# symek/facedeform

Measured on AMD Instinct MI355X. Metric: deformed Mverts/sec at 256 ctrl pts, 1/2/4/8 MI355X vs host-CPU ref, higher is better.
Workload: dtype f32

## Files before the change

### facedeform_amd/_build.py

```python
from __future__ import annotations

import os
import shutil
import subprocess

_PKG = os.path.dirname(os.path.abspath(__file__))
_ROOT = os.path.dirname(_PKG)
CSRC = os.path.join(_PKG, "csrc")
LIB_DIR = os.path.join(_PKG, "lib")
LIB_PATH = os.path.join(LIB_DIR, "libfacedeform_hip.so")
SOURCES = ["fd_eval.hip", "fd_eval_shared.hip", "fd_build.hip", "fd_nullspace.hip", "fd_build_reg.hip", "fd_build_ml_shared.hip", "fd_build_qnn_shared.hip", "fd_capi.hip", "fd_morph.hip", "fd_capture.hip", "fd_vectors.hip", "fd_invert.hip", "fd_adjoint.hip", "fd_adjoint_points.hip", "fd_adjoint_shot.hip", "fd_adjoint_points_shot.hip", "fd_gram.hip", "fd_bake.hip", "fd_vectors_shared.hip", "fd_eval_shared64.hip", "fd_vectors_shared64.hip", "fd_eval_shared_ml.hip", "fd_vectors_shared_ml.hip", "fd_eval_shared_ml64.hip", "fd_vectors_shared_ml64.hip", "fd_sop_host.cpp"]
EXTRA_FLAGS = {"fd_eval.hip": ["-mllvm", "-amdgpu-mfma-vgpr-form"],
               "fd_eval_shared.hip": ["-fno-slp-vectorize"],
               "fd_eval_shared_ml.hip": ["-fno-slp-vectorize"],
               "fd_vectors_shared64.hip": ["-mllvm", "-disable-machine-licm"],
               "fd_vectors_shared_ml64.hip": ["-mllvm", "-disable-machine-licm"],
               "fd_adjoint_shot.hip": ["-mllvm", "-disable-machine-licm"],
               "fd_adjoint_points.hip": ["-mllvm", "-disable-machine-licm"],
               "fd_adjoint_points_shot.hip": ["-mllvm", "-disable-machine-licm"]}
HEADERS = [os.path.join(CSRC, "fd_internal.h"), os.path.join(CSRC, "fd_tuning.h"), os.path.join(CSRC, "fd_pack.h"), os.path.join(CSRC, "fd_eval_common.h"), os.path.join(CSRC, "fd_transport.h"), os.path.join(CSRC, "fd_eval_point.h"), os.path.join(CSRC, "fd_shot_launch.h"), os.path.join(CSRC, "fd_vectors_shot.h"), os.path.join(CSRC, "fd_shared64.h"), os.path.join(CSRC, "fd_shared_ml64.h"), os.path.join(CSRC, "fd_shared_ml.h"), os.path.join(CSRC, "fd_shared_common.h"), os.path.join(CSRC, "fd_shared_plan.h"), os.path.join(CSRC, "fd_shared_solve.h"), os.path.join(CSRC, "fd_shot_dev.h"), os.path.join(CSRC, "fd_fit_host.h"), os.path.join(CSRC, "fd_owned.h"), os.path.join(CSRC, "fd_operator.h"), os.path.join(CSRC, "fd_adjoint_points_shot.h"), os.path.join(CSRC, "fd_bake_plan.h"), os.path.join(_ROOT, "include", "facedeform_hip.h")]


def hipcc_path() -> str:
    for cand in (os.environ.get("HIPCC"), shutil.which("hipcc"), "/opt/rocm/bin/hipcc"):
        if cand and os.path.exists(cand):
            return cand
    raise RuntimeError("hipcc not found (set HIPCC or install ROCm)")


def is_stale() -> bool:
    if not os.path.exists(LIB_PATH):
        return True
    t = os.path.getmtime(LIB_PATH)
    deps = [os.path.join(CSRC, s) for s in SOURCES] + HEADERS
    return any(os.path.getmtime(d) > t for d in deps)


def build(force: bool = False, verbose: bool = False) -> str:
    if not force and not is_stale():
        return LIB_PATH
    os.makedirs(LIB_DIR, exist_ok=True)
    obj_dir = os.path.join(_PKG, "build")
    os.makedirs(obj_dir, exist_ok=True)
    cc = hipcc_path()
    common = ["--offload-arch=gfx950", "-O3", "-std=c++17", "-fPIC", "-ffp-contract=off", "-I", os.path.join(_ROOT, "include")]
    common += os.environ.get("FD_EXTRA_HIPCC_FLAGS", "").split()
    objs = []
    procs = []
    for src in SOURCES:
        obj = os.path.join(obj_dir, os.path.splitext(src)[0] + ".o")
        objs.append(obj)
        cmd = [cc] + common + EXTRA_FLAGS.get(src, []) + ["-x", "hip", "-c", os.path.join(CSRC, src), "-o", obj]
        if verbose:
            print(" ".join(cmd))
        procs.append((src, subprocess.Popen(cmd, stdout=subprocess.PIPE, stderr=subprocess.STDOUT)))
    for src, p in procs:
        out, _ = p.communicate()
        if p.returncode != 0:
            raise RuntimeError(f"hipcc failed on {src}:\n{out.decode(errors='replace')}")
    tmp = LIB_PATH + ".tmp"
    link = [cc, "--offload-arch=gfx950", "-shared", "-fPIC", "-o", tmp] + objs
    subprocess.check_call(link)
    os.replace(tmp, LIB_PATH)
    return LIB_PATH


if __name__ == "__main__":
    print(build(force=True, verbose=True))
```

### facedeform_amd/csrc/fd_build_reg.hip

```cpp
#include <cstdio>
#include <cstdlib>

#include "fd_internal.h"
#include "fd_pack.h"

namespace fd {

namespace {

typedef double double4_t __attribute__((ext_vector_type(4)));

constexpr double kEps = 2.220446049250313e-16;
constexpr int kRegThreads = 512;
constexpr int kRegWaves = kRegThreads / 64;
constexpr int kMaxBlocks = 16;
constexpr int kWorkers = 7;
constexpr int kSlots = 20;
constexpr int kPitch = 17;
constexpr int kTileLds = 16 * kPitch;

__device__ __forceinline__ double readlane_f64(double v, int src_lane)
{
    const long long b = __double_as_longlong(v);
    const unsigned lo = (unsigned)__builtin_amdgcn_readlane((int)(b & 0xffffffffll), src_lane);
    const unsigned hi = (unsigned)__builtin_amdgcn_readlane((int)(b >> 32), src_lane);
    return __longlong_as_double((long long)(((unsigned long long)hi << 32) | lo));
}

__device__ __forceinline__ int opaque_s(int v)
{
    asm volatile("" : "+s"(v));
    return v;
}

template <int CTRL>
__device__ __forceinline__ double dpp_f64(double v)
{
    const long long b = __double_as_longlong(v);
    const unsigned lo = (unsigned)__builtin_amdgcn_update_dpp(0, (int)(b & 0xffffffffll), CTRL, 0xf, 0xf, false);
    const unsigned hi = (unsigned)__builtin_amdgcn_update_dpp(0, (int)(b >> 32), CTRL, 0xf, 0xf, false);
    return __longlong_as_double((long long)(((unsigned long long)hi << 32) | lo));
}
__device__ __forceinline__ double wave_sum(double v)
{
    const double4_t zero = {0.0, 0.0, 0.0, 0.0};
    const double4_t d = __builtin_amdgcn_mfma_f64_16x16x4f64(v, 1.0, zero, 0, 0, 0);
    const double t = (d[0] + d[1]) + (d[2] + d[3]);
    const double4_t e = __builtin_amdgcn_mfma_f64_16x16x4f64(t, 1.0, zero, 0, 0, 0);
    return e[0];
}
__device__ __forceinline__ double wave_max(double v)
{
    double o;
    o = dpp_f64<0x121>(v); v = o > v ? o : v;
    o = dpp_f64<0x122>(v); v = o > v ? o : v;
    o = dpp_f64<0x124>(v); v = o > v ? o : v;
    o = dpp_f64<0x128>(v); v = o > v ? o : v;
    const double a = readlane_f64(v, 0), b = readlane_f64(v, 16), c = readlane_f64(v, 32), d = readlane_f64(v, 48);
    const double ab = a > b ? a : b, cd = c > d ? c : d;
    return ab > cd ? ab : cd;
}

__device__ __forceinline__ void wave_lds_sync()
{
    __builtin_amdgcn_fence(__ATOMIC_RELEASE, "wavefront");
    __builtin_amdgcn_wave_barrier();
    __builtin_amdgcn_fence(__ATOMIC_ACQUIRE, "wavefront");
}

__device__ __forceinline__ double rsqrt_nr(double d)
{
    const double y0 = __builtin_amdgcn_rsq(d);
    const double t = d * y0;
    const double e = fma(-t, y0, 1.0);
    double p = fma(e, 0.375, 0.5);
    p = p * e;
    return fma(y0, p, y0);
}

__device__ __forceinline__ double log_pos(double x)
{
    double m = __builtin_amdgcn_frexp_mant(x);
    int e = __builtin_amdgcn_frexp_exp(x);
    if (m < 0.70710678118654752) { m *= 2.0; e -= 1; }
    const double num = m - 1.0, den = m + 1.0;
    double r = __builtin_amdgcn_rcp(den);
    r = fma(fma(-den, r, 1.0), r, r);
// ... 45 lines not shown
    L.cen = p; p += 3 * kRows;
    L.V = p; p += 4 * kRows;
    L.W = p; p += 4 * kRows;
    L.F = p; p += 3 * kRows;
    L.B21 = p; p += 4 * kRows;
    L.small = p; p += kSmallDoubles;
    const size_t overlay = (size_t)kMaxBlocks * kTileLds + (size_t)(kMaxBlocks + 1) * kTileLds;
    const size_t ypart = (size_t)kRegWaves * 4 * kRows;
    L.minv = p; L.P = p + (size_t)kMaxBlocks * kTileLds; L.ypart = p;
    p += overlay > ypart ? overlay : ypart;
    L.scr = p; p += (size_t)kRegWaves * 2 * kTileLds;
    L.Z = p; p += 3 * 256;
    L.Y = p; p += 3 * 256;
    L.stat = p; p += 8;
    L.D = p; p += kTileLds;
    L.tab = reinterpret_cast<int *>(p);
    L.flag = L.tab + 300;
    return L;
}

__device__ __forceinline__ double4_t factor_invert_tile(double4_t Tt, int lane, double &piv)
{
    const int c = lane & 15, g = lane >> 4;
    piv = 0.0;
    double4_t U;
#pragma unroll
    for (int i = 0; i < 4; ++i) U[i] = (g + 4 * i == c) ? 1.0 : 0.0;
#pragma unroll
    for (int b = 0; b < 4; ++b) {
        double s[4][4];
#pragma unroll
        for (int p = 0; p < 4; ++p)
#pragma unroll
            for (int q = 0; q <= p; ++q) s[p][q] = readlane_f64(Tt[b], 4 * b + q + 16 * p);
        double l[4][4], inv[4], dk[4];
#pragma unroll
        for (int k = 0; k < 4; ++k) {
            double d = s[k][k];
#pragma unroll
            for (int e = 0; e < k; ++e) d = fma(-l[k][e], l[k][e], d);
            dk[k] = d;
            inv[k] = rsqrt_nr(d);
#pragma unroll
            for (int p = k + 1; p < 4; ++p) {
                double v = s[p][k];
#pragma unroll
                for (int e = 0; e < k; ++e) v = fma(-l[p][e], l[k][e], v);
                l[p][k] = v * inv[k];
            }
        }
#pragma unroll
        for (int k = 0; k < 4; ++k) piv = c == 4 * b + k ? dk[k] : piv;
        double m[4][4];
#pragma unroll
        for (int q = 0; q < 4; ++q) {
            m[q][q] = inv[q];
#pragma unroll
            for (int p = q + 1; p < 4; ++p) {
                double v = 0.0;
#pragma unroll
                for (int e = q; e < p; ++e) v = fma(l[p][e], m[e][q], v);
                m[p][q] = -v * inv[p];
            }
        }
        double aop = 0.0;
#pragma unroll
        for (int p = 0; p < 4; ++p)
#pragma unroll
            for (int q = 0; q <= p; ++q) aop = (c == p && g == q) ? m[p][q] : aop;
        const double4_t zero = {0.0, 0.0, 0.0, 0.0};
        const double4_t rt = __builtin_amdgcn_mfma_f64_16x16x4f64(aop, Tt[b], zero, 0, 0, 0);
        const double4_t ru = __builtin_amdgcn_mfma_f64_16x16x4f64(aop, U[b], zero, 0, 0, 0);
        const double mult = c > 4 * b + 3 ? -rt[0] : 0.0;
        Tt = __builtin_amdgcn_mfma_f64_16x16x4f64(mult, rt[0], Tt, 0, 0, 0);
        U = __builtin_amdgcn_mfma_f64_16x16x4f64(mult, ru[0], U, 0, 0, 0);
        U[b] = ru[0];
        Tt[b] = rt[0];
    }
    return U;
}

constexpr int kAff = 64;
struct PackLds {
    const double *cen, *dlt, *sol, *aff;
    const float *dl_global;
    double R;
    int sing, dup;
    __device__ __forceinline__ double centre(int j, int q) const { return cen[3 * j + q]; }
    __device__ __forceinline__ bool has_delta() const { return true; }
    __device__ __forceinline__ double delta(int j, int q) const { return dlt ? dlt[3 * j + q] : (double)dl_global[3 * j + q]; }
    __device__ __forceinline__ double weight(int j, int c) const { return sol[c * 256 + j]; }
    __device__ __forceinline__ double affine(int cc, int k, int, int T) const { return k < T ? aff[3 * k + cc] : 0.0; }
    __device__ __forceinline__ double radius(int) const { return R; }
    __device__ __forceinline__ int sing_flag() const { return sing; }
    __device__ __forceinline__ int dup_flag() const { return dup; }
};

__device__ __forceinline__ double lds_where(bool cond, const double *p, int i_true)
{
    const double v = p[cond ? i_true : 0];
    return cond ? v : 0.0;
}

__device__ __forceinline__ void assemble_tile(const double *cen, int I, int J, int c, int g, int M, int kind, double lambda, double inv_r2,
                                              double (&e)[4], double &amax_w, bool &dup)
{
    const int col = 16 * J + c;
    const double cx = cen[3 * col], cy = cen[3 * col + 1], cz = cen[3 * col + 2];
    double d2[4];
#pragma unroll
    for (int i = 0; i < 4; ++i) {
        const int row = 16 * I + g + 4 * i;
        const double dx = cen[3 * row] - cx, dy = cen[3 * row + 1] - cy, dz = cen[3 * row + 2] - cz;
        d2[i] = dx * dx + dy * dy + dz * dz;
    }
    if (kind == FD_KERNEL_THIN_PLATE) {
#pragma unroll
        for (int i = 0; i < 4; ++i) {
            const bool pos = d2[i] > 0.0;
            const double lg = log_pos(pos ? d2[i] : 1.0);
            e[i] = pos ? 0.5 * d2[i] * lg : 0.0;
        }
    } else {
#pragma unroll
        for (int i = 0; i < 4; ++i) e[i] = phi_reg(kind, d2[i], inv_r2);
    }
#pragma unroll
    for (int i = 0; i < 4; ++i) {
        const int row = 16 * I + g + 4 * i;
        const bool real = row < M && col < M;
        if (row == col) e[i] += lambda;
        else if (d2[i] == 0.0 && real) dup = true;
        if (!real) e[i] = 0.0;
        const double ae = fabs(e[i]);
        amax_w = ae > amax_w ? ae : amax_w;
    }
}

__device__ __forceinline__ void reflect_wave(const RegLds &L, int M, int T, int lane)
{
    bool singular = false;
    double cn[4] = {0.0, 0.0, 0.0, 0.0};
    double v[4][4], f[4][3];
#pragma unroll
    for (int q = 0; q < 4; ++q) {
        const int i = lane + 64 * q;
        const bool in = i < M;
        const int ic = in ? i : 0;
        const double p[4] = {1.0, L.cen[3 * ic], L.cen[3 * ic + 1], L.cen[3 * ic + 2]};
#pragma unroll
        for (int t = 0; t < 4; ++t) {
            v[q][t] = (in && t < T) ? p[t] : 0.0;
            if (in) cn[t] = fma(v[q][t], v[q][t], cn[t]);
        }
#pragma unroll
        for (int e = 0; e < 3; ++e) { const double d = L.F[e * kRows + ic]; f[q][e] = in ? d : 0.0; }
    }
#pragma unroll
    for (int t = 0; t < 4; ++t) cn[t] = wave_sum(cn[t]);
#pragma unroll
    for (int k = 0; k < 4; ++k) {
        if (k >= T) break;
        const int piv = M - 1 - k;
        const int pl = __builtin_amdgcn_readfirstlane(piv & 63), pq = __builtin_amdgcn_readfirstlane(piv >> 6);
        double rowv[4], rowf[3];
#define FD_PIVOT_ROW(Q) { _Pragma("unroll") for (int t = 0; t < 4; ++t) rowv[t] = readlane_f64(v[Q][t], pl); \
                          _Pragma("unroll") for (int e = 0; e < 3; ++e) rowf[e] = readlane_f64(f[Q][e], pl); }
        if (pq == 0) FD_PIVOT_ROW(0) else if (pq == 1) FD_PIVOT_ROW(1) else if (pq == 2) FD_PIVOT_ROW(2) else FD_PIVOT_ROW(3)
#undef FD_PIVOT_ROW
        double acc[7] = {0.0, 0.0, 0.0, 0.0, 0.0, 0.0, 0.0};
        double x[4];
#pragma unroll
        for (int q = 0; q < 4; ++q) {
// ... 101 lines not shown

__device__ __forceinline__ void gram_wave(const RegLds &L, int M, int lane)
{
    double Sm[16];
#pragma unroll
    for (int q = 0; q < 16; ++q) Sm[q] = 0.0;
#pragma unroll
    for (int q = 0; q < 4; ++q) {
        const int i = lane + 64 * q;
        if (i < M) {
#pragma unroll
            for (int a = 0; a < 4; ++a)
#pragma unroll
                for (int b = 0; b < 4; ++b) Sm[4 * a + b] = fma(L.V[4 * i + a], L.W[4 * i + b], Sm[4 * a + b]);
        }
    }
#pragma unroll
    for (int q = 0; q < 16; ++q) Sm[q] = wave_sum(Sm[q]);
    double Tm[16], ST[16], Gm[16];
#pragma unroll
    for (int q = 0; q < 16; ++q) Tm[q] = L.small[kTm + q];
#pragma unroll
    for (int a = 0; a < 4; ++a)
#pragma unroll
        for (int b = 0; b < 4; ++b) {
            double v = 0.0;
#pragma unroll
            for (int cc = 0; cc < 4; ++cc) v = fma(0.5 * (Sm[4 * a + cc] + Sm[4 * cc + a]), Tm[4 * cc + b], v);
            ST[4 * a + b] = v;
        }
#pragma unroll
    for (int a = 0; a < 4; ++a)
#pragma unroll
        for (int b = 0; b < 4; ++b) {
            double v = 0.0;
#pragma unroll
            for (int cc = 0; cc < 4; ++cc) v = fma(Tm[4 * cc + a], ST[4 * cc + b], v);
            Gm[4 * a + b] = v;
        }
#pragma unroll
    for (int a = 0; a < 4; ++a)
#pragma unroll
        for (int b = a + 1; b < 4; ++b) { const double m = 0.5 * (Gm[4 * a + b] + Gm[4 * b + a]); Gm[4 * a + b] = m; Gm[4 * b + a] = m; }
    if (lane < 16) {
        double v = 0.0;
#pragma unroll
        for (int q = 0; q < 16; ++q) v = lane == q ? Gm[q] : v;
        L.small[kGm + lane] = v;
    }
}

__device__ __forceinline__ void w_row(const RegLds &L, int i)
{
    double y[4], v[4], w[4];
#pragma unroll
    for (int t = 0; t < 4; ++t) { y[t] = L.W[4 * i + t]; v[t] = L.V[4 * i + t]; }
#pragma unroll
    for (int b = 0; b < 4; ++b) {
        double z = 0.0, h = 0.0;
#pragma unroll
        for (int a = 0; a < 4; ++a) { z = fma(y[a], L.small[kTm + 4 * a + b], z); h = fma(v[a], L.small[kGm + 4 * a + b], h); }
        w[b] = fma(-0.5, h, z);
    }
#pragma unroll
    for (int t = 0; t < 4; ++t) L.W[4 * i + t] = w[t];
}

__device__ __forceinline__ int tile_owner(int I, int J)
{
    constexpr unsigned long long kOffsets = 0x8a3ad602e31bull;
    auto w0 = [](int K) { return (K + 1 + (int)((kOffsets >> (3 * K)) & 7ull)) % kWorkers; };
    if (I == J) return J == 0 ? 0 : w0(J - 1);
    const int j = I - J - 1;
    return j == 0 ? w0(J) : (w0(J) + 1 + (j - 1) % 6) % kWorkers;
}

constexpr int kFacTiles = kMaxBlocks * (kMaxBlocks + 1) / 2;
constexpr size_t kFacL = 0, kFacMinv = (size_t)kFacTiles * 256, kFacV = kFacMinv + (size_t)kMaxBlocks * kTileLds, kFacB21 = kFacV + 4 * kRows,
                 kFacSmall = kFacB21 + 4 * kRows, kFacMeta = kFacSmall + kSmallDoubles, kFacDoubles = kFacMeta + 8;

constexpr int kFront1Tiles = kWorkers;
constexpr int kFront2Tiles = kRegWaves;
constexpr size_t kFrV = 0, kFrF = 4 * kRows, kFrB21 = 7 * kRows, kFrSmall = 11 * kRows, kFrMeta = kFrSmall + kSmallDoubles,
                 kFrTile = kFrMeta + 8, kFrY = kFrTile + 2 * (size_t)(kMaxBlocks * (kMaxBlocks + 1) / 2);
__host__ __device__ inline size_t reg_front_doubles(int M)
{
    const int nbk = (M + 15) / 16;
    return kFrY + (size_t)(nbk * (nbk + 1) / 2) * 128;
}
__device__ __forceinline__ int tile_number(int I, int J, int nbk) { return J * nbk - J * (J - 1) / 2 + (I - J); }

constexpr int kFrontMaxTpw = 4;
__global__ __launch_bounds__(kRegThreads) void k_reg_front1(const BatchSlot *tab, const PointSrc src, int use_src, int M, int T, int kind,
                                                             double lambda, double gauss_R, int tpw)
{
    const BatchSlot &slot = tab[blockIdx.z];
    __shared__ __attribute__((aligned(16))) double s_mem[10 * kRows + kSmallDoubles + 8 + kWorkers * kTileLds];
    RegLds L{};
    L.cen = s_mem; L.V = L.cen + 3 * kRows; L.F = L.V + 4 * kRows; L.small = L.F + 3 * kRows; L.stat = L.small + kSmallDoubles; L.scr = L.stat + 8;
    const int tid = threadIdx.x, lane = tid & 63;
    const int wave = __builtin_amdgcn_readfirstlane(tid >> 6);
    const int c = lane & 15, g = lane >> 4;
    const int nbk = (M + 15) / 16, ntiles = nbk * (nbk + 1) / 2;
    const bool first = blockIdx.x == 0;
    {
        const float *rest = use_src ? src.rest[blockIdx.z] : slot.rest;
        const float *delta = use_src ? src.delta[blockIdx.z] : slot.delta;
        for (int i = tid; i < M; i += kRegThreads) {
#pragma unroll
            for (int q = 0; q < 3; ++q) {
                const float r = rest[3 * i + q], d = delta[3 * i + q];
                L.cen[3 * i + q] = (double)r;
                L.F[q * kRows + i] = (double)d;
                if (first) {
                    slot.centres[3 * i + q] = (double)r;
                    if (use_src) { slot.rest[3 * i + q] = r; slot.delta[3 * i + q] = d; }
                }
            }
            if (first) slot.radii[i] = gauss_R;
        }
        for (int e = tid; e < 4 * kRows; e += kRegThreads) {
            if (e >= 4 * M || T == 0) L.V[e] = 0.0;
            if (e < 3 * kRows && e % kRows >= M) L.F[e] = 0.0;
            if (e < 3 * kRows && e >= 3 * M) L.cen[e] = 0.0;
        }
        if (tid < kSmallDoubles) L.small[tid] = 0.0;
        if (tid == 0) L.stat[3] = 0.0;
    }
    __syncthreads();
    gdouble *fr = as_global(slot.ns);
    double e[kFrontMaxTpw][4];
    int tI[kFrontMaxTpw], tJ[kFrontMaxTpw];
    bool have[kFrontMaxTpw];
    if (wave < kWorkers) {
        gdouble *stage = as_global(slot.A);
        const double inv_r2 = 1.0 / (gauss_R * gauss_R);
#pragma unroll
        for (int t = 0; t < kFrontMaxTpw; ++t) {
            const int q = ((int)blockIdx.x * tpw + t) * kFront1Tiles + wave;
            have[t] = t < tpw && q < ntiles;
            tI[t] = tJ[t] = 0;
#pragma unroll
            for (int i = 0; i < 4; ++i) e[t][i] = 0.0;
            if (have[t]) {
                int r = q, J = 0;
                while (r >= nbk - J) { r -= nbk - J; ++J; }
                tI[t] = J + r; tJ[t] = J;
                double amax_w = 0.0;
                bool dup = false;
                assemble_tile(L.cen, tI[t], tJ[t], c, g, M, kind, lambda, inv_r2, e[t], amax_w, dup);
#pragma unroll
                for (int i = 0; i < 4; ++i) stage[((size_t)q * 4 + i) * 64 + lane] = e[t][i];
                amax_w = wave_max(amax_w);
                const bool any_dup = __any(dup);
                if (lane == 0) { fr[kFrTile + 2 * q] = amax_w; fr[kFrTile + 2 * q + 1] = any_dup ? 1.0 : 0.0; }
            }
        }
    } else {
#pragma unroll
        for (int t = 0; t < kFrontMaxTpw; ++t) have[t] = false;
        if (T > 0) reflect_wave(L, M, T, lane);
    }
    __threadfence_block();
    __syncthreads();
    if (T > 0) {
#pragma unroll
        for (int t = 0; t < kFrontMaxTpw; ++t) {
            if (!have[t]) continue;
            const int q = ((int)blockIdx.x * tpw + t) * kFront1Tiles + wave;
            const int I = tI[t], J = tJ[t];
            gdouble *yq = fr + kFrY + (size_t)q * 128;
            double *sb = L.scr + (size_t)wave * kTileLds;
            if (I != J) {
                wave_lds_sync();
#pragma unroll
                for (int i = 0; i < 4; ++i) sb[(g + 4 * i) * kPitch + c] = e[t][i];
            }
            {
                double4_t acc = {0.0, 0.0, 0.0, 0.0};
#pragma unroll
                for (int s2 = 0; s2 < 4; ++s2) {
                    const double b = lds_where(c < 4, L.V, 4 * (16 * I + 4 * s2 + g) + c);
                    acc = __builtin_amdgcn_mfma_f64_16x16x4f64(e[t][s2], b, acc, 0, 0, 0);
                }
                if (c < 4) {
#pragma unroll
                    for (int i = 0; i < 4; ++i) yq[(g + 4 * i) * 4 + c] = acc[i];
                }
            }
            if (I != J) {
                wave_lds_sync();
                double4_t acc = {0.0, 0.0, 0.0, 0.0};
#pragma unroll
                for (int s2 = 0; s2 < 4; ++s2) {
                    const double a = sb[c * kPitch + 4 * s2 + g];
                    const double b = lds_where(c < 4, L.V, 4 * (16 * J + 4 * s2 + g) + c);
                    acc = __builtin_amdgcn_mfma_f64_16x16x4f64(a, b, acc, 0, 0, 0);
                }
                if (c < 4) {
#pragma unroll
                    for (int i = 0; i < 4; ++i) yq[64 + (g + 4 * i) * 4 + c] = acc[i];
                }
            }
        }
    }
    if (first && wave == kWorkers) {
        for (int x = lane; x < 4 * kRows; x += 64) fr[kFrV + x] = L.V[x];
        for (int x = lane; x < 3 * kRows; x += 64) fr[kFrF + x] = L.F[x];
        for (int x = lane; x < kSmallDoubles; x += 64) fr[kFrSmall + x] = L.small[x];
        if (lane == 0) fr[kFrMeta + 2] = L.stat[3];
    }
}

__global__ __launch_bounds__(kRegThreads) void k_reg_front2(const BatchSlot *tab, int M, int T, int tpw)
{
    const BatchSlot &slot = tab[blockIdx.z];
    __shared__ __attribute__((aligned(16))) double s_mem[8 * kRows + kSmallDoubles];
    RegLds L{};
    L.V = s_mem; L.W = L.V + 4 * kRows; L.small = L.W + 4 * kRows;
    const int tid = threadIdx.x, lane = tid & 63;
    const int wave = __builtin_amdgcn_readfirstlane(tid >> 6);
    const int c = lane & 15, g = lane >> 4;
    const int n1 = M - T;
    const int nbk = (M + 15) / 16, ntiles = nbk * (nbk + 1) / 2;
    gdouble *fr = as_global(slot.ns);
    for (int x = tid; x < 4 * kRows; x += kRegThreads) {
        L.V[x] = fr[kFrV + x];
        const int i = x >> 2, t = x & 3, r = i >> 4, row = i & 15;
        double y = 0.0;
        if (T > 0 && r < nbk) {
            gcdouble *yp = fr + kFrY + row * 4 + t;
            double v[kMaxBlocks];
#pragma unroll
            for (int k = 0; k < kMaxBlocks; ++k) {
                const int kk = k < nbk ? k : nbk - 1;
                const size_t at = kk < r ? (size_t)tile_number(r, kk, nbk) * 128 + 64 : (size_t)tile_number(kk, r, nbk) * 128;
                v[k] = yp[at];
            }
#pragma unroll
            for (int k = 0; k < kMaxBlocks; ++k) y += k < nbk ? v[k] : 0.0;
        }
        L.W[x] = y;
    }
    if (tid < kSmallDoubles) L.small[tid] = fr[kFrSmall + tid];
    if (blockIdx.x == 0 && wave == 1) {
        double amax = 0.0, dup = 0.0;
        for (int q = lane; q < ntiles; q += 64) {
            const double a = fr[kFrTile + 2 * q], d = fr[kFrTile + 2 * q + 1];
            amax = a > amax ? a : amax; dup = d > dup ? d : dup;
        }
        amax = wave_max(amax); dup = wave_max(dup);
        if (lane == 0) { fr[kFrMeta + 0] = amax; fr[kFrMeta + 1] = dup; }
    }
    __syncthreads();
    if (T > 0) {
        if (wave == 0) gram_wave(L, M, lane);
        __syncthreads();
        if (tid < kRows) w_row(L, tid);
        __syncthreads();
    }
    gdouble *stage = as_global(slot.A);
    for (int t = 0; t < tpw; ++t) {
        const int q = ((int)blockIdx.x * tpw + t) * kFront2Tiles + wave;
        if (q >= ntiles) break;
        int I = 0, J = 0;
        {
            int r = q;
            while (r >= nbk - J) { r -= nbk - J; ++J; }
            I = J + r;
        }
        double4_t S;
#pragma unroll
        for (int i = 0; i < 4; ++i) S[i] = stage[((size_t)q * 4 + i) * 64 + lane];
        if (T > 0) {
            const int ri = 16 * I + c, rj = 16 * J + c;
            const double vi = L.V[4 * ri + g], wi = L.W[4 * ri + g];
            const double vj = L.V[4 * rj + g], wj = L.W[4 * rj + g];
            S = __builtin_amdgcn_mfma_f64_16x16x4f64(-vi, wj, S, 0, 0, 0);
            S = __builtin_amdgcn_mfma_f64_16x16x4f64(-wi, vj, S, 0, 0, 0);
        }
#pragma unroll
        for (int i = 0; i < 4; ++i) {
            const int row = 16 * I + g + 4 * i, col = 16 * J + c;
            if (row >= n1 && row < M && col < n1) fr[kFrB21 + 4 * col + (M - 1 - row)] = S[i];
            if (row >= n1 || col >= n1) S[i] = row == col ? 1.0 : 0.0;
            stage[((size_t)q * 4 + i) * 64 + lane] = S[i];
        }
    }
}

template <bool FRONT>
__global__ __launch_bounds__(kRegThreads) void k_build_reg(const BatchSlot *tab, const PointSrc src, int use_src, int M, int T, int npad,
                                                            int kind, int Mpad, double lambda, double gauss_R, unsigned long long *stamps,
                                                            double *fac)
{
    const BatchSlot &slot = tab[blockIdx.z];
    extern __shared__ __attribute__((aligned(16))) double dyn_lds[];
    const RegLds L = carve(dyn_lds, M);
    const int tid = threadIdx.x, lane = tid & 63;
    const int wave = __builtin_amdgcn_readfirstlane(tid >> 6);
    const bool worker = wave < kWorkers;
    const int c = lane & 15, g = lane >> 4;
    const int n1 = M - T;
    const int nbk = (M + 15) / 16;
    const int nb = (n1 + 15) / 16;
    DevModel FD_GLOBAL *model = as_global(slot.model);
    unsigned long long st_prev = stamps ? __builtin_amdgcn_s_memtime() : 0ull;
    int st_k = 0;
#define FD_RSTAMP() if (stamps && blockIdx.z == 0 && tid == 0) { const unsigned long long t_ = __builtin_amdgcn_s_memtime(); stamps[st_k] = t_ - st_prev; atomicAdd(&stamps[84 + st_k], t_ - st_prev); if (st_k == 0) atomicAdd(&stamps[83], 1ull); ++st_k; st_prev = t_; }
    __builtin_amdgcn_s_setprio(3);

    const int ntiles = nbk * (nbk + 1) / 2;
    int nmine = 0;
    if (worker) {
        if (lane < kSlots) L.tab[wave * kSlots + lane] = 0xffff;
        wave_lds_sync();
        for (int q0 = 0; q0 < ntiles; q0 += 64) {
            int q = q0 + lane, J = 0;
            const bool in = q < ntiles;
            while (in && q >= nbk - J) { q -= nbk - J; ++J; }
            const int I = J + q;
            const bool mine = in && tile_owner(I, J) == wave;
            const unsigned long long mask = __ballot(mine);
            const int rank = nmine + __popcll(mask & ((1ull << lane) - 1ull));
            if (mine) L.tab[wave * kSlots + rank] = I | (J << 8) | ((q0 + lane) << 16);
            nmine += __popcll(mask);
        }
        nmine = __builtin_amdgcn_readfirstlane(nmine);
    }
    if constexpr (!FRONT) {
        gcdouble *fr = as_global(slot.ns);
        static_assert(4 * kRows == 2 * kRegThreads, "two entries per thread");
        double lv[2], lb[2], lf[2], ls[2], lc[2], ld[2];
#pragma unroll
        for (int h = 0; h < 2; ++h) {
            const int e = tid + kRegThreads * h;
            lv[h] = fr[kFrV + e];
            lb[h] = fr[kFrB21 + e];
            lf[h] = fr[kFrF + (e < 3 * kRows ? e : 0)];
            ls[h] = fr[kFrSmall + (e < kSmallDoubles ? e : 0)];
            lc[h] = slot.centres[e < 3 * M ? e : 0];
            ld[h] = (double)slot.delta[e < 3 * M ? e : 0];
        }
#pragma unroll
        for (int h = 0; h < 2; ++h) {
            const int e = tid + kRegThreads * h;
            L.V[e] = lv[h];
            L.B21[e] = lb[h];
            if (e < 3 * kRows) L.F[e] = lf[h];
            if (e < kSmallDoubles) L.small[e] = ls[h];
            if (e < 3 * M) { L.cen[e] = lc[h]; L.scr[e] = ld[h]; }
        }
    } else {
        const float *rest = use_src ? src.rest[blockIdx.z] : slot.rest;
        const float *delta = use_src ? src.delta[blockIdx.z] : slot.delta;
        for (int i = tid; i < M; i += kRegThreads) {
#pragma unroll
            for (int q = 0; q < 3; ++q) {
                const float r = rest[3 * i + q], d = delta[3 * i + q];
                L.cen[3 * i + q] = (double)r;
                L.F[q * kRows + i] = (double)d;
                slot.centres[3 * i + q] = (double)r;
                if (use_src) { slot.rest[3 * i + q] = r; slot.delta[3 * i + q] = d; }
            }
            slot.radii[i] = gauss_R;
        }
        for (int e = tid; e < 4 * kRows; e += kRegThreads) {
            if (e >= 4 * M) { L.V[e] = 0.0; L.W[e] = 0.0; L.B21[e] = 0.0; }
            if (e < 3 * kRows && e % kRows >= M) L.F[e] = 0.0;
            if (e < 3 * kRows && e >= 3 * M) L.cen[e] = 0.0;
        }
    }
    if (tid == 0) { L.stat[0] = INFINITY; L.stat[1] = 0.0; L.stat[2] = 0.0; L.stat[3] = FRONT ? 0.0 : as_global(slot.ns)[kFrMeta + 2]; L.flag[0] = 0; L.flag[1] = 0; L.flag[2] = 0; L.flag[3] = 0; }
    __syncthreads();
    int ijv = 0xffff;
    if (worker && lane < kSlots) ijv = L.tab[wave * kSlots + lane];
    const int ivI = ijv & 0xff, ivJ = (ijv >> 8) & 0xff;
    auto slots_where = [&](bool cond) -> unsigned { return (unsigned)__builtin_amdgcn_readfirstlane((int)(unsigned)__ballot(cond && lane < kSlots)); };
    const unsigned m_matrix = slots_where(ivI < kMaxBlocks);
#define tI(t) (opaque_s(__builtin_amdgcn_readlane(ijv, t)) & 0xff)
#define tJ(t) ((opaque_s(__builtin_amdgcn_readlane(ijv, t)) >> 8) & 0xff)
#define FD_SLOT(m, t) (((m) >> (t)) & 1u)
    FD_RSTAMP()

    if constexpr (FRONT) {
    if (worker) {
        gdouble *stage = as_global(slot.A);
        const double inv_r2 = 1.0 / (gauss_R * gauss_R);
        double amax_w = 0.0;
        bool dup = false;
#pragma nounroll
        for (int t = 0; t < nmine; ++t) {
            const int ij = __builtin_amdgcn_readfirstlane(L.tab[wave * kSlots + t]);
            const int I = ij & 0xff, J = (ij >> 8) & 0xff, q = ij >> 16;
            double e[4];
            assemble_tile(L.cen, I, J, c, g, M, kind, lambda, inv_r2, e, amax_w, dup);
#pragma unroll
            for (int i = 0; i < 4; ++i) {
                stage[((size_t)q * 4 + i) * 64 + lane] = e[i];
            }
        }
        amax_w = wave_max(amax_w);
        const bool any_dup = __any(dup);
        if (lane == 0) { L.ypart[wave] = amax_w; L.ypart[kRegWaves + wave] = any_dup ? 1.0 : 0.0; }
    } else if (T > 0) {
        reflect_wave(L, M, T, lane);
    }
    __threadfence_block();
    __syncthreads();
    }
    FD_RSTAMP()
    double amax = 0.0;
    bool dup_any = false;
    if constexpr (FRONT) {
#pragma unroll
        for (int w = 0; w < kWorkers; ++w) { amax = L.ypart[w] > amax ? L.ypart[w] : amax; dup_any = dup_any || L.ypart[kRegWaves + w] != 0.0; }
    } else {
        amax = as_global(slot.ns)[kFrMeta + 0];
        dup_any = as_global(slot.ns)[kFrMeta + 1] != 0.0;
    }
    double4_t S[kSlots];
    {
        gcdouble *stage = as_global(slot.A);
#pragma unroll
        for (int t = 0; t < kSlots; ++t) {
            const int q = __builtin_amdgcn_readlane(ijv, t) >> 16;
            S[t] = (double4_t){0.0, 0.0, 0.0, 0.0};
            if (FD_SLOT(m_matrix, t)) {
#pragma unroll
                for (int i = 0; i < 4; ++i) S[t][i] = stage[((size_t)q * 4 + i) * 64 + lane];
            }
        }
    }
    if constexpr (FRONT) {
// ... 308 lines not shown
    }
    for (int I = nb - 1; I >= 1; --I) {
        const unsigned m_row = slots_where(ivI == I && ivJ < I);
        const bool next_mine = slots_where(ivI == I && ivJ == I - 1) != 0u;
#pragma unroll
        for (int t = 0; t < kSlots; ++t) {
            if (FD_SLOT(m_row, t)) {
                double4_t acc = {0.0, 0.0, 0.0, 0.0};
                double ya[4];
#pragma unroll
                for (int s = 0; s < 4; ++s) ya[s] = lds_where(c < 3, L.Y, c * 256 + 16 * I + 4 * s + g);
                __builtin_amdgcn_sched_group_barrier(0x100, 4, 0);
                __builtin_amdgcn_sched_group_barrier(0x002, 8, 0);
                __builtin_amdgcn_sched_group_barrier(0x008, 4, 0);
#pragma unroll
                for (int s = 0; s < 4; ++s) acc = __builtin_amdgcn_mfma_f64_16x16x4f64(ya[s], S[t][s], acc, 0, 0, 0);
                if (g < 3) L.Z[g * 256 + 16 * tJ(t) + c] -= acc[0];
            }
        }
        if (next_mine) { wave_lds_sync(); solve_block(I - 1); }
        __syncthreads();
    }
    FD_RSTAMP()

    if (!worker) {
        double q12[12];
#pragma unroll
        for (int e = 0; e < 12; ++e) q12[e] = 0.0;
        double xr[4][3];
#pragma unroll
        for (int q = 0; q < 4; ++q) {
            const int i = lane + 64 * q;
            const bool in = i < n1;
            xr[q][0] = in ? L.Y[i] : 0.0; xr[q][1] = in ? L.Y[256 + i] : 0.0; xr[q][2] = in ? L.Y[512 + i] : 0.0;
            if (in && T > 0) {
#pragma unroll
                for (int k = 0; k < 4; ++k) {
                    const double b = k < T ? L.B21[4 * i + k] : 0.0;
                    q12[3 * k] = fma(b, xr[q][0], q12[3 * k]); q12[3 * k + 1] = fma(b, xr[q][1], q12[3 * k + 1]); q12[3 * k + 2] = fma(b, xr[q][2], q12[3 * k + 2]);
                }
            }
        }
        if (T > 0) {
#pragma unroll
            for (int e = 0; e < 12; ++e) q12[e] = wave_sum(q12[e]);
        }
        double a[4][3] = {};
#pragma unroll
        for (int k = 3; k >= 0; --k) {
            if (k >= T) continue;
#pragma unroll
            for (int e = 0; e < 3; ++e) {
                double v = L.small[kG + 3 * k + e] - q12[3 * k + e];
#pragma unroll
                for (int c2 = k + 1; c2 < 4; ++c2) if (c2 < T) v = fma(-L.small[kR + 4 * k + c2], a[c2][e], v);
                a[k][e] = v / L.small[kR + 4 * k + k];
            }
        }
#pragma unroll
        for (int k = 3; k >= 0; --k) {
            if (k >= T) continue;
            const int piv = M - 1 - k;
            const double tau = L.small[kTau + k];
            double d[3] = {0.0, 0.0, 0.0}, v[4];
#pragma unroll
            for (int q = 0; q < 4; ++q) {
                const int i = lane + 64 * q;
                v[q] = i <= piv ? L.V[4 * i + k] : 0.0;
#pragma unroll
                for (int e = 0; e < 3; ++e) d[e] = fma(v[q], xr[q][e], d[e]);
            }
#pragma unroll
            for (int e = 0; e < 3; ++e) d[e] = wave_sum(d[e]);
#pragma unroll
            for (int q = 0; q < 4; ++q)
#pragma unroll
                for (int e = 0; e < 3; ++e) xr[q][e] = fma(-tau * d[e], v[q], xr[q][e]);
        }
        gdouble *X = as_global(slot.X);
#pragma unroll
        for (int q = 0; q < 4; ++q) {
            const int i = lane + 64 * q;
            if (i < M) { X[i] = xr[q][0]; X[(size_t)npad + i] = xr[q][1]; X[2 * (size_t)npad + i] = xr[q][2]; }
            if (i < M) { L.Y[i] = xr[q][0]; L.Y[256 + i] = xr[q][1]; L.Y[512 + i] = xr[q][2]; }
        }
        if (lane < 12) {
            double v = 0.0;
#pragma unroll
            for (int k = 0; k < 4; ++k)
#pragma unroll
                for (int e = 0; e < 3; ++e) v = lane == 3 * k + e ? a[k][e] : v;
            L.small[kAff + lane] = v;
        }
        for (int r = M + lane; r < npad; r += 64) {
#pragma unroll
            for (int e = 0; e < 3; ++e) {
                double v = 0.0;
#pragma unroll
                for (int k = 0; k < 4; ++k) v = (r - M == k && k < T) ? a[k][e] : v;
                X[(size_t)e * npad + r] = v;
            }
        }
        if (lane == 0) {
            model->terminationtype = 0;
            model->dup_flag = dup_any ? 1 : 0;
            model->sing_flag = (L.stat[2] != 0.0 || L.stat[3] != 0.0) ? 1 : 0;
            L.stat[4] = (L.stat[2] != 0.0 || L.stat[3] != 0.0) ? 1.0 : 0.0;
            L.stat[5] = dup_any ? 1.0 : 0.0;
            model->iterations = M + T;
            model->amax_bits = (unsigned long long)__double_as_longlong(amax);
            model->pivmin_bits = (unsigned long long)__double_as_longlong(L.stat[0]);
            model->pivmax_bits = (unsigned long long)__double_as_longlong(L.stat[1]);
        }
    }
    __threadfence_block();
    __syncthreads();
    FD_RSTAMP()
    if (tid >= 256) return;
    {
        const PackLds in{L.cen, FRONT ? nullptr : L.scr, L.Y, L.small + kAff, slot.delta, gauss_R, L.stat[4] != 0.0 ? 1 : 0, L.stat[5] != 0.0 ? 1 : 0};
        packing::pack_body_from(in, slot, npad, M, Mpad, T, kind, 0, 0);
    }
    FD_RSTAMP()
    if (kind == FD_KERNEL_THIN_PLATE) {
        __syncthreads();
        for (int tile = tid >> 6; tile < Mpad / 16; tile += 4) packing::pack_tiles_body(slot, Mpad, tile, lane);
    }
    FD_RSTAMP()
#undef FD_RSTAMP
#undef tI
#undef tJ
#undef FD_SLOT
}

__global__ __launch_bounds__(256) void k_resolve_reg(const BatchSlot *tab, const PointSrc src, int use_src, int M, int T, int npad, int kind,
                                                      int Mpad, double gauss_R, const double *fac)
{
    const int fi = 1 + (int)blockIdx.z;
    const BatchSlot &slot = tab[fi];
    __shared__ double s_minv[kMaxBlocks * kTileLds];
    __shared__ double s_V[4 * kRows], s_B21[4 * kRows], s_small[kSmallDoubles];
    __shared__ double s_f[3 * kRows];
    __shared__ double s_blk[3 * 16];
    __shared__ double s_red[4 * 12];
    __shared__ double s_g[12], s_a[12];
    const int tid = threadIdx.x, lane = tid & 63;
    const int n1 = M - T, nb = (n1 + 15) / 16, nbk = (M + 15) / 16;
    gcdouble *fg = as_global(fac);
    DevModel FD_GLOBAL *model = as_global(slot.model);
    auto tile_q = [&](int I, int J) { return J * nbk - J * (J - 1) / 2 + (I - J); };
    for (int e = tid; e < kMaxBlocks * kTileLds; e += 256) s_minv[e] = fg[kFacMinv + e];
    for (int e = tid; e < 4 * kRows; e += 256) { s_V[e] = fg[kFacV + e]; s_B21[e] = fg[kFacB21 + e]; }
    if (tid < kSmallDoubles) s_small[tid] = fg[kFacSmall + tid];
    {
        const float *rest = use_src ? src.rest[fi] : slot.rest;
        const float *delta = use_src ? src.delta[fi] : slot.delta;
        for (int i = tid; i < kRows; i += 256) {
#pragma unroll
            for (int q = 0; q < 3; ++q) {
                double d = 0.0;
                if (i < M) {
                    const float r = rest[3 * i + q], dl = delta[3 * i + q];
                    d = (double)dl;
                    slot.centres[3 * i + q] = (double)r;
                    if (use_src) { slot.rest[3 * i + q] = r; slot.delta[3 * i + q] = dl; }
                }
                s_f[q * kRows + i] = d;
            }
            if (i < M) slot.radii[i] = gauss_R;
        }
    }
    __syncthreads();
    const int i0 = tid;
    for (int k = 0; k < T; ++k) {
        const int piv = M - 1 - k;
        const double v = s_V[4 * i0 + k];
        double d[3] = {v * s_f[i0], v * s_f[kRows + i0], v * s_f[2 * kRows + i0]};
        packing::block_reduce_many<3, false>(d, s_red, tid);
        const double tau = s_small[kTau + k];
#pragma unroll
        for (int e = 0; e < 3; ++e) {
            const double fv = fma(-tau * d[e], v, s_f[e * kRows + i0]);
            if (i0 == piv) { s_g[3 * k + e] = fv; s_f[e * kRows + i0] = 0.0; }
            else if (i0 < piv) s_f[e * kRows + i0] = fv;
        }
        __syncthreads();
    }
    {
        const int r = tid, I = r >> 4, rr = r & 15;
        double cur[16], nxt[16];
        auto fetch = [&](int K, double (&dst)[16]) {
            if (I > K && I < nb) {
                gcdouble *p = fg + kFacL + ((size_t)tile_q(I, K) * 4 + (rr >> 2)) * 64 + 16 * (rr & 3);
#pragma unroll
                for (int k = 0; k < 16; ++k) dst[k] = p[k];
            } else {
#pragma unroll
                for (int k = 0; k < 16; ++k) dst[k] = 0.0;
            }
        };
        fetch(0, cur);
        for (int K = 0; K < nb; ++K) {
            if (K + 1 < nb) fetch(K + 1, nxt);
            if (tid < 48) {
                const int e = tid >> 4, n = tid & 15;
                const double *mk = s_minv + (size_t)K * kTileLds;
                double z = 0.0;
#pragma unroll
                for (int k = 0; k < 16; ++k) z = fma(s_f[e * kRows + 16 * K + k], mk[n * kPitch + k], z);
                s_blk[e * 16 + n] = z;
            }
            __syncthreads();
            if (tid < 48) s_f[(tid >> 4) * kRows + 16 * K + (tid & 15)] = s_blk[tid];
            if (I > K && I < nb) {
#pragma unroll
// ... 73 lines not shown
#pragma unroll
                    for (int c2 = k + 1; c2 < 4; ++c2) if (c2 < T) v = fma(-s_small[kR + 4 * k + c2], a[c2][e], v);
                    a[k][e] = v / s_small[kR + 4 * k + k];
                }
            }
#pragma unroll
            for (int k = 0; k < 4; ++k)
#pragma unroll
                for (int e = 0; e < 3; ++e) s_a[3 * k + e] = a[k][e];
        }
        for (int k = T - 1; k >= 0; --k) {
            const int piv = M - 1 - k;
            const double v = i0 <= piv ? s_V[4 * i0 + k] : 0.0;
            double d[3] = {v * xr[0], v * xr[1], v * xr[2]};
            packing::block_reduce_many<3, false>(d, s_red, tid);
            const double tau = s_small[kTau + k];
#pragma unroll
            for (int e = 0; e < 3; ++e) xr[e] = fma(-tau * d[e], v, xr[e]);
        }
        __syncthreads();
        gdouble *X = as_global(slot.X);
        if (i0 < M) { X[i0] = xr[0]; X[(size_t)npad + i0] = xr[1]; X[2 * (size_t)npad + i0] = xr[2]; }
        for (int rrow = M + tid; rrow < npad; rrow += 256) {
#pragma unroll
            for (int e = 0; e < 3; ++e) X[(size_t)e * npad + rrow] = (rrow - M < T) ? s_a[3 * (rrow - M) + e] : 0.0;
        }
        if (tid == 0) {
            model->terminationtype = 0;
            model->dup_flag = fg[kFacMeta + 1] != 0.0 ? 1 : 0;
            model->sing_flag = fg[kFacMeta + 2] != 0.0 ? 1 : 0;
            model->iterations = M + T;
            model->amax_bits = (unsigned long long)__double_as_longlong(fg[kFacMeta + 0]);
            model->pivmin_bits = (unsigned long long)__double_as_longlong(fg[kFacMeta + 3]);
            model->pivmax_bits = (unsigned long long)__double_as_longlong(fg[kFacMeta + 4]);
        }
    }
    __threadfence_block();
    __syncthreads();
    packing::pack_body(slot, npad, M, Mpad, T, kind, 0, 0);
    if (kind == FD_KERNEL_THIN_PLATE) {
        __syncthreads();
        for (int tile = tid >> 6; tile < Mpad / 16; tile += 4) packing::pack_tiles_body(slot, Mpad, tile, lane);
    }
}

}

size_t reg_factor_doubles() { return kFacDoubles; }

bool reg_applicable(int kind, int term, double lambda, int M)
{
    return M <= 16 * kMaxBlocks && spd_applicable(kind, term, lambda, M);
}

hipError_t reg_build_init()
{
    static bool done[64] = {};
    int dev = 0;
    hipError_t e = hipGetDevice(&dev);
    if (e != hipSuccess) return e;
    if (dev >= 0 && dev < 64 && done[dev]) return hipSuccess;
    e = hipFuncSetAttribute((const void *)k_build_reg<true>, hipFuncAttributeMaxDynamicSharedMemorySize,
                            (int)(sizeof(double) * reg_lds_doubles(16 * kMaxBlocks)));
    if (e == hipSuccess)
        e = hipFuncSetAttribute((const void *)k_build_reg<false>, hipFuncAttributeMaxDynamicSharedMemorySize,
                                (int)(sizeof(double) * reg_lds_doubles(16 * kMaxBlocks)));
    if (e == hipSuccess && dev >= 0 && dev < 64) done[dev] = true;
    return e;
}

hipError_t launch_build_reg_shared(const BuildBuffers &b, hipStream_t stream, const PointSrc *src, hipEvent_t ev_mid, double *fac)
{
    static const PointSrc none{};
    if (ev_mid) (void)hipEventRecord(ev_mid, stream);
    const size_t lds = sizeof(double) * reg_lds_doubles(b.M);
    hipLaunchKernelGGL(k_build_reg<true>, dim3(1, 1, 1), dim3(kRegThreads), lds, stream, b.d_slots, src ? *src : none, src ? 1 : 0, b.M, b.T,
                       b.npad, b.kind, b.Mpad, b.lambda, b.gauss_R, (unsigned long long *)nullptr, fac);
    if (b.nbatch > 1)
        hipLaunchKernelGGL(k_resolve_reg, dim3(1, 1, (unsigned)b.nbatch - 1), dim3(256), 0, stream, b.d_slots, src ? *src : none, src ? 1 : 0,
                           b.M, b.T, b.npad, b.kind, b.Mpad, b.gauss_R, (const double *)fac);
    return hipGetLastError();
}

hipError_t launch_build_reg(const BuildBuffers &b, hipStream_t stream, const PointSrc *src, hipEvent_t ev_mid)
{
    static const PointSrc none{};
    const unsigned nbatch = (unsigned)b.nbatch;
    if (ev_mid) (void)hipEventRecord(ev_mid, stream);
    const size_t lds = sizeof(double) * reg_lds_doubles(b.M);
    static unsigned long long *d_stamps = nullptr;
    hipStreamCaptureStatus cs = hipStreamCaptureStatusNone;
    static const bool stamps_env = tuning_env("FD_REG_STAMPS") != nullptr;
    static const bool stamps_late = stamps_env && atoi(tuning_env("FD_REG_STAMPS")) == 2;
    const bool want_stamps = stamps_env && hipStreamIsCapturing(stream, &cs) == hipSuccess && cs == hipStreamCaptureStatusNone;
    if (want_stamps && !d_stamps) { (void)hipMalloc((void **)&d_stamps, 96 * sizeof(unsigned long long)); (void)hipMemset(d_stamps, 0, 96 * sizeof(unsigned long long)); }
    const bool split = b.reg_front != 0 && reg_front_doubles(b.M) <= ns_doubles(b.M);
    if (split) {
        const int nbk = (b.M + 15) / 16, ntiles = nbk * (nbk + 1) / 2;
        const int cus = (int)device_cus();
        auto tiles_per_wave = [&](int per_wg) {
            int tpw = 1;
            while (tpw < kFrontMaxTpw && ((ntiles + per_wg * tpw - 1) / (per_wg * tpw)) * (int)nbatch > cus) ++tpw;
            return tpw;
        };
        const int tpw1 = tiles_per_wave(kFront1Tiles), tpw2 = tiles_per_wave(kFront2Tiles);
        hipLaunchKernelGGL(k_reg_front1, dim3((unsigned)((ntiles + kFront1Tiles * tpw1 - 1) / (kFront1Tiles * tpw1)), 1, nbatch), dim3(kRegThreads), 0, stream,
                           b.d_slots, src ? *src : none, src ? 1 : 0, b.M, b.T, b.kind, b.lambda, b.gauss_R, tpw1);
        hipLaunchKernelGGL(k_reg_front2, dim3((unsigned)((ntiles + kFront2Tiles * tpw2 - 1) / (kFront2Tiles * tpw2)), 1, nbatch), dim3(kRegThreads), 0, stream,
                           b.d_slots, b.M, b.T, tpw2);
        hipLaunchKernelGGL(k_build_reg<false>, dim3(1, 1, nbatch), dim3(kRegThreads), lds, stream, b.d_slots, none, 0, b.M, b.T,
                           b.npad, b.kind, b.Mpad, b.lambda, b.gauss_R, want_stamps ? d_stamps : nullptr, (double *)nullptr);
    } else
    hipLaunchKernelGGL(k_build_reg<true>, dim3(1, 1, nbatch), dim3(kRegThreads), lds, stream, b.d_slots, src ? *src : none, src ? 1 : 0, b.M, b.T,
                       b.npad, b.kind, b.Mpad, b.lambda, b.gauss_R, want_stamps ? d_stamps : nullptr, (double *)nullptr);
    if (want_stamps && d_stamps && stamps_late) {
        static bool registered = false;
        static unsigned long long *d_keep = nullptr;
        d_keep = d_stamps;
        if (!registered) {
            registered = true;
            atexit([] {
                unsigned long long h[96];
                if (d_keep && hipDeviceSynchronize() == hipSuccess && hipMemcpy(h, d_keep, sizeof(h), hipMemcpyDeviceToHost) == hipSuccess && h[83]) {
                    fprintf(stderr, "[k_build_reg stamps, MEAN over %llu launches (no read-back per launch): table | assembly | tile loads | reflectors | KV | W + rotation | Cholesky | back substitution | recovery | pack]\n  ", h[83]);
                    for (int q = 0; q < 10; ++q) fprintf(stderr, " %llu", h[84 + q] / h[83]);
                    fprintf(stderr, "\n");
                }
            });
        }
    } else if (want_stamps && d_stamps) {
        unsigned long long h[80];
        (void)hipStreamSynchronize(stream);
        if (hipMemcpy(h, d_stamps, sizeof(h), hipMemcpyDeviceToHost) == hipSuccess) {
            fprintf(stderr, "[k_build_reg stamps, shader cycles: table | assembly | tile loads | reflectors + Q^T f | Y = K V | W + rotation + B21 | Cholesky | back substitution | recovery | pack]\n  ");
            for (int q = 0; q < 10; ++q) fprintf(stderr, " %llu", h[q]);
            fprintf(stderr, "\n   Cholesky steps (cycles since its start: inverse K in LDS | panel K in LDS, as wave 0 sees them):");
            for (int q = 16; q < 48; ++q) fprintf(stderr, "%s%llu", (q - 16) % 2 ? " " : "\n     ", h[q]);
            fprintf(stderr, "\n");
        }
    }
    return hipGetLastError();
}

}
```

### facedeform_amd/csrc/fd_capi.hip

```cpp
#include <algorithm>
#include <atomic>
#include <chrono>
#include <cmath>
#include <cstdarg>
#include <cstdio>
#include <cstdlib>
#include <cstring>
#include <initializer_list>
#include <new>
#include <vector>

#include "fd_fit_host.h"
#include "fd_internal.h"
#include "fd_owned.h"
#include "fd_shared_plan.h"

using namespace fd;
using namespace fd_fit;

struct GraphKey {
    int M, kind, term, nparams;
    double params[4];
    const void *A, *rest, *rec32;
};
// ... 58 lines not shown
    bool status_inflight = false;
    int sticky_rc = FD_OK;

    int64_t cap_N = 0;
    DevBuf<float> d_P, d_dist2, d_fall;
    DevBuf<float> d_tu, d_tv, d_nrm;
    DevBuf<float> d_vec, d_vecP;
    DevBuf<int> d_iters;
    DevBuf<double> d_adj;
    DevBuf<double> d_adjp;
    DevBuf<double> d_gram;
    DevBuf<double> d_bake, d_bakeout;
    DevBuf<double> d_adjs;
    DevBuf<float> d_gshot;
    size_t cap_hgshot = 0;
    float *h_gshot = nullptr;
    int64_t mesh_N = 0, mesh_cap = 0;
    bool mesh_has_dist2 = false, mesh_has_frames = false;
    DevBuf<float> m_P, m_dist2, m_tu, m_tv, m_nrm;
    DevBuf<float> m_out, m_fall;

    Event ev0, ev_mid, ev1;

    GraphExec build_exec;
    bool use_graph = true;
    GraphKey graph_key{}, resolve_key{};
    char err[512] = {0};
};

struct ShotScratch {
    DevBuf<void> d;
    Event consumed_ev;
    bool consumed = false;
    Event eval_ev;
    bool eval_pending = false;
};

struct fd_batch {
    int n = 0;
    int device = 0;
    fd_ctx *ctxs[kMaxBatch] = {};
    uint64_t gens[kMaxBatch] = {};
    DevBuf<BatchSlot> d_slots;
    PointSrc src{};
    bool have_src = false;
    Event ev0, ev_mid, ev1;
    GraphExec exec;
    bool use_graph = true;
    GraphKey key{};
    hipStream_t waited_stream = nullptr;
    Event status_ev;
    struct SharedSet {
        DevBuf<void> d_wtiles, d_frames;
        Event packed_ev;
        Event eval_ev;
        hipEvent_t eval_done = nullptr;
        bool eval_pending = false;
    } sets[2];
    Pinned<int> h_mismatch;
    int eval_cus = 0;
    int shared_factor = 0;
    DevBuf<double> d_fac;
    int last_shared_factor = 0;
    DevBuf<void> d_mlfac;
    int shared_lu = 0;
    DevBuf<void> d_qnnfac;
    bool qnn_slot_ready = false;
    int qnn_slot_M = 0, qnn_slot_npad = 0;
    int cur_set = 0;
    bool packed_valid = false;
    bool prepared = false;
    unsigned long long prep_gen[kMaxBatch] = {0};
    float *prep_P_out[kMaxBatch] = {nullptr};
    float *prep_fall[kMaxBatch] = {nullptr};
    bool prep_has_fall = false;
    Event fallback_ev;
    ShotScratch s64;
    ShotScratch sml;
    ShotScratch sml64;
    ShotScratch sadjp;
    Event group_ev;
    bool lean = false;
    hipEvent_t consumed_override = nullptr;
    char err[512] = {0};
};


static thread_local char g_err[512] = {0};

static void set_err(fd_ctx *ctx, const char *fmt, ...)
{
    char *dst = ctx ? ctx->err : g_err;
    va_list ap;
    va_start(ap, fmt);
    vsnprintf(dst, 512, fmt, ap);
    va_end(ap);
}

static hipStream_t cur_stream(fd_ctx *ctx)
{
    if (ctx->stream_) return ctx->stream_;
    if (!ctx->own_stream && ctx->own_stream.create() != hipSuccess) (void)hipGetLastError();
    return ctx->own_stream;
}

#define FD_HIP(ctx, call)                                                               \
    do {                                                                                \
        hipError_t e_ = (call);                                                         \
        if (e_ != hipSuccess) {                                                         \
            set_err(ctx, "%s failed: %s (%s:%d)", #call, hipGetErrorString(e_), __FILE__, __LINE__); \
            return FD_E_DEVICE;                                                         \
        }                                                                               \
    } while (0)

static int use_device(fd_ctx *ctx)
{
    int cur = -1;
    FD_HIP(ctx, hipGetDevice(&cur));
    if (cur != ctx->device) FD_HIP(ctx, hipSetDevice(ctx->device));
    return FD_OK;
}

constexpr bool kGrow = true;
template <typename T>
static int dev_alloc(fd_ctx *ctx, DevBuf<T> &b, size_t count, bool grow = false)
{
    const hipError_t e = grow ? b.grow(count) : b.alloc(count);
    if (e == hipSuccess) return FD_OK;
    set_err(ctx, "hipMalloc(%zu bytes) failed: %s", (count ? count : 1) * sizeof(T), hipGetErrorString(e));
    return FD_E_NOMEM;
}

static int order_of(const fd_ctx *ctx) { return ctx->M + term_cols(ctx->term); }
static int ml_layers(const fd_ctx *ctx) { return ctx->kind == FD_KERNEL_GAUSSIAN_ML ? (int)ctx->params[1] : 0; }
static int model_centres(const fd_ctx *ctx) { return ctx->kind == FD_KERNEL_GAUSSIAN_ML ? ctx->M * ml_layers(ctx) : ctx->M; }
static int eval_kind(const fd_ctx *ctx) { return ctx->kind == FD_KERNEL_GAUSSIAN_ML ? FD_KERNEL_GAUSSIAN_QNN : ctx->kind; }
static int record_layers(const fd_ctx *ctx) { return ctx->kind == FD_KERNEL_GAUSSIAN_ML ? ml_layers(ctx) : ctx->imported_layers; }

static int ensure_records_capacity(fd_ctx *ctx, int n)
{
    int rc;
    if (n > ctx->cap_records) {
        const int npad = round_up(n, kRecPad);
        if ((rc = dev_alloc(ctx, ctx->d_centres, (size_t)n * 3))) return rc;
        if ((rc = dev_alloc(ctx, ctx->d_radii, (size_t)n))) return rc;
        if ((rc = dev_alloc(ctx, ctx->d_W, (size_t)(n + 4) * 3))) return rc;
        if ((rc = dev_alloc(ctx, ctx->d_rec32, (size_t)npad))) return rc;
        if ((rc = dev_alloc(ctx, ctx->d_rec64, (size_t)npad))) return rc;
        if ((rc = dev_alloc(ctx, ctx->d_tiles, (size_t)npad / 16))) return rc;
        if ((rc = dev_alloc(ctx, ctx->d_tiles16, (size_t)npad / 16))) return rc;
        ctx->cap_records = n;
    }
    return FD_OK;
}

static int ensure_model_capacity(fd_ctx *ctx, int M)
{
    int rc;
    if (M > ctx->cap_M) {
        if ((rc = dev_alloc(ctx, ctx->d_rest, (size_t)M * 3))) return rc;
        if ((rc = dev_alloc(ctx, ctx->d_delta, (size_t)M * 3))) return rc;
        if ((rc = dev_alloc(ctx, ctx->d_ns, ns_doubles(M)))) return rc;
        ctx->cap_M = M;
    }
    return ensure_records_capacity(ctx, M);
}
// ... 1614 lines not shown
    va_end(ap);
}

fd_batch *fd_batch_create(fd_ctx *const *ctxs, int n)
{
    if (!ctxs || n <= 0 || n > kMaxBatch) { set_err(nullptr, "fd_batch_create: need 1..%d contexts", kMaxBatch); return nullptr; }
    for (int i = 0; i < n; ++i) {
        if (!ctxs[i] || ctxs[i]->device != ctxs[0]->device) { set_err(nullptr, "fd_batch_create: contexts must exist and share one device"); return nullptr; }
        for (int j = 0; j < i; ++j)
            if (ctxs[j] == ctxs[i]) { set_err(nullptr, "fd_batch_create: context listed twice"); return nullptr; }
    }
    fd_batch *b = new (std::nothrow) fd_batch();
    if (!b) { set_err(nullptr, "fd_batch_create: out of host memory"); return nullptr; }
    b->n = n;
    b->device = ctxs[0]->device;
    for (int i = 0; i < n; ++i) b->ctxs[i] = ctxs[i];
    bool ok = hipSetDevice(b->device) == hipSuccess;
    ok = ok && b->d_slots.alloc((size_t)n) == hipSuccess;
    ok = ok && b->ev0.create(hipEventDefault) == hipSuccess && b->ev_mid.create(hipEventDefault) == hipSuccess &&
         b->ev1.create(hipEventDefault) == hipSuccess;
    ok = ok && b->status_ev.create(hipEventDisableTiming) == hipSuccess;
    ok = ok && b->h_mismatch.alloc(1, hipHostMallocMapped) == hipSuccess;
    if (ok) *b->h_mismatch = 0;
    if (!ok) {
        set_err(nullptr, "fd_batch_create: device resource allocation failed: %s", hipGetErrorString(hipGetLastError()));
        fd_batch_destroy(b);
        return nullptr;
    }
    return b;
}

void fd_batch_destroy(fd_batch *b)
{
    if (!b) return;
    (void)hipSetDevice(b->device);
    for (int i = 0; i < b->n; ++i) {
        fd_ctx *c = b->ctxs[i];
        if (c && c->wait_event == b->ev1) {
            if (c->wait_stream) (void)hipStreamSynchronize(c->wait_stream);
            c->wait_event = nullptr; c->wait_stream = nullptr; c->wait_batch = nullptr;
        }
        if (c && c->tev0 == b->ev0) { c->tev0 = c->ev0; c->tev_mid = c->ev_mid; c->tev1 = c->ev1; }
        if (c && (c->status_poll == b->status_ev || c->status_poll == b->ev1)) { c->status_poll = c->status_ev; c->status_inflight = false; }
    }
    delete b;
}

const char *fd_batch_last_error(const fd_batch *b) { return b ? b->err : g_err; }

int fd_batch_set_points_dev(fd_batch *b, const float *const *d_rest_xyz, const float *const *d_delta_xyz, int M)
{
    if (!b || !d_rest_xyz || !d_delta_xyz) return FD_E_INVALID;
    if (M <= 0 || M + 4 > kMaxOrder) { batch_err(b, "fd_batch_set_points_dev: M = %d outside 1..%d", M, kMaxOrder - 4); return FD_E_INVALID; }
    b->prepared = false;
    if (b->h_mismatch && *b->h_mismatch != 0) {
        const int who = *b->h_mismatch - 1;
        *b->h_mismatch = 0;
        batch_err(b, "shared-rig evaluation of the previous group: context %d was built on other rest points than context 0 (same "
                     "address, other contents); its frame was passed through", who);
        return FD_E_INVALID;
    }
    for (int i = 0; i < b->n; ++i)
        if (!d_rest_xyz[i] || !d_delta_xyz[i]) { batch_err(b, "fd_batch_set_points_dev: null array for context %d", i); return FD_E_INVALID; }
    for (int i = 0; i < b->n; ++i) {
        fd_ctx *c = b->ctxs[i];
        int rc = use_device(c);
        if (!rc) rc = ensure_model_capacity(c, M);
        if (rc) { batch_err(b, "context %d: %s", i, c->err); return rc; }
        c->M = M;
        c->points_set = true;
        c->built = false;
        c->build_pending = false;
        c->have_factor = false;
        c->deltas_only = false;
        c->rest_src = d_rest_xyz[i];
        c->rig_build_id = 0;
        b->src.rest[i] = d_rest_xyz[i];
        b->src.delta[i] = d_delta_xyz[i];
    }
    b->have_src = true;
    return FD_OK;
}

int fd_batch_build_async(fd_batch *b, void *hip_stream)
{
    if (!b) return FD_E_INVALID;
    b->prepared = false;
    fd_ctx *c0 = b->ctxs[0];
    int rc = use_device(c0);
    if (rc) { batch_err(b, "%s", c0->err); return rc; }
    hipStream_t stream = hip_stream ? (hipStream_t)hip_stream : cur_stream(c0);
    for (int i = 0; i < b->n; ++i) {
        fd_ctx *c = b->ctxs[i];
        if (!c->points_set) { batch_err(b, "fd_batch_build: context %d has no control points", i); return FD_E_INVALID; }
        c->imported_layers = 0;
        if (!same_model(c, c0)) {
            batch_err(b, "fd_batch_build: context %d differs from context 0 in M, kernel, parameters or term", i);
            return FD_E_INVALID;
        }
    }
    const int npad = round_up(order_of(c0), 32);
    bool table_stale = false;
    for (int i = 0; i < b->n; ++i) {
        fd_ctx *c = b->ctxs[i];
        const bool grew = npad > c->cap_npad;
        if ((rc = ensure_solver_capacity(c, npad)) || (rc = ensure_records_capacity(c, model_centres(c))) || (rc = sync_slot(c))) {
            batch_err(b, "context %d: %s", i, c->err);
            return rc;
        }
        if (grew) {
            const size_t cols = (size_t)c->cap_npad + kRhsCols + 16;
            hipError_t e = hipMemsetAsync(c->d_A, 0, sizeof(double) * (size_t)c->cap_npad * cols, stream);
            if (e != hipSuccess) { batch_err(b, "hipMemsetAsync failed: %s", hipGetErrorString(e)); return FD_E_DEVICE; }
        }
        if (b->gens[i] != c->alloc_gen) table_stale = true;
    }
    if (table_stale) {
        b->qnn_slot_ready = false;
        BatchSlot tab[kMaxBatch];
        for (int i = 0; i < b->n; ++i) { tab[i] = b->ctxs[i]->h_slot; b->gens[i] = b->ctxs[i]->alloc_gen; }
        hipError_t e = hipMemcpy(b->d_slots, tab, sizeof(BatchSlot) * (size_t)b->n, hipMemcpyHostToDevice);
        if (e != hipSuccess) { batch_err(b, "slot table upload failed: %s", hipGetErrorString(e)); return FD_E_DEVICE; }
    }
    BuildBuffers bb;
    choose_build(b->ctxs, b->n, bb);
    bb.d_slots = b->d_slots;
    bb.nbatch = b->n;
    if (bb.reg && reg_build_init() != hipSuccess) { (void)hipGetLastError(); bb.reg = 0; }
    bb.reg_front = (b->eval_cus <= 0 || b->eval_cus >= (int)device_cus()) ? 1 : 0;
    bb.group_panels = b->n >= 4 ? 1 : 0;

    bool same_rest_launch = b->have_src;
    for (int i = 1; i < b->n && same_rest_launch; ++i) same_rest_launch = b->src.rest[i] == b->src.rest[0];
    bool shared_ml = b->shared_factor != 0 && bb.ml_layers > 0 && same_rest_launch && ml_shared_applies(bb.M, bb.ml_layers, b->n);
    if (shared_ml && ml_shared_init() != hipSuccess) { (void)hipGetLastError(); shared_ml = false; }
    if (shared_ml && b->d_mlfac.grow(ml_shared_scratch_bytes(bb)) != hipSuccess) { (void)hipGetLastError(); shared_ml = false; }
    bool shared_qnn = b->shared_lu != 0 && c0->kind == FD_KERNEL_GAUSSIAN_QNN && bb.ml_layers == 0 && bb.nopivot && !bb.spd &&
                      bb.npad <= 1024 && bb.M >= bb.T && same_rest_launch && qnn_shared_applies(bb.M, b->n);
    for (int i = 0; i < b->n && shared_qnn; ++i) shared_qnn = b->ctxs[i]->solver == FD_SOLVER_AUTO;
    if (shared_qnn && qnn_shared_init() != hipSuccess) { (void)hipGetLastError(); shared_qnn = false; }
    if (shared_qnn && qnn_shared_scratch_bytes(bb) > b->d_qnnfac.cap) {
        b->qnn_slot_ready = false;
        if (b->d_qnnfac.grow(qnn_shared_scratch_bytes(bb)) != hipSuccess) { (void)hipGetLastError(); shared_qnn = false; }
    }

    const GraphKey key = graph_key(c0, (bb.spd << 9) | (bb.small << 10) | (bb.reg << 11) | (bb.nopivot << 12), false);
    if (!bb.reg && !shared_ml && !shared_qnn && b->use_graph &&
        ensure_graph(stream, &b->exec, &b->key, key, [&] { return launch_build(bb, stream, nullptr); }) != hipSuccess)
        b->use_graph = false;
#define FD_BHIP(call)                                                                         \
    do {                                                                                      \
        hipError_t e_ = (call);                                                               \
        if (e_ != hipSuccess) { batch_err(b, "%s failed: %s", #call, hipGetErrorString(e_)); return FD_E_DEVICE; } \
    } while (0)
    const bool shared_fac_ok = same_rest_launch;
    bool shared_fac = b->shared_factor != 0 && bb.reg && shared_fac_ok && b->n > 1;
    if (shared_fac && !b->d_fac && b->d_fac.alloc(reg_factor_doubles()) != hipSuccess) {
        (void)hipGetLastError(); shared_fac = false;
    }
    b->last_shared_factor = (shared_fac || shared_ml || shared_qnn) ? 1 : 0;
    if (!b->lean) FD_BHIP(hipEventRecord(b->ev0, stream));
    if (shared_fac) {
        FD_BHIP(launch_build_reg_shared(bb, stream, &b->src, nullptr, b->d_fac));
        b->have_src = false;
    } else if (bb.reg) {
        FD_BHIP(launch_build_reg(bb, stream, b->have_src ? &b->src : nullptr, nullptr));
        b->have_src = false;
    } else {
    FD_BHIP(launch_prepare(bb, stream, b->have_src ? &b->src : nullptr));
    b->have_src = false;
    if (shared_ml) {
        FD_BHIP(hipEventRecord(b->ev_mid, stream));
        FD_BHIP(launch_build_ml_shared(bb, stream, b->d_mlfac));
    } else if (shared_qnn) {
        FD_BHIP(hipEventRecord(b->ev_mid, stream));
        const bool fill = !(b->qnn_slot_ready && b->qnn_slot_M == bb.M && b->qnn_slot_npad == bb.npad);
        b->qnn_slot_ready = false;
        FD_BHIP(launch_build_qnn_shared(bb, stream, b->d_qnnfac, fill));
        b->qnn_slot_ready = true; b->qnn_slot_M = bb.M; b->qnn_slot_npad = bb.npad;
    } else if (b->use_graph && b->exec) {
        FD_BHIP(hipEventRecord(b->ev_mid, stream));
        FD_BHIP(hipGraphLaunch(b->exec, stream));
    } else {
        FD_BHIP(launch_build(bb, stream, b->ev_mid));
    }
    }
    if (!b->lean) FD_BHIP(hipEventRecord(b->ev1, stream));
    b->waited_stream = nullptr;
#undef FD_BHIP
    static std::atomic<uint64_t> build_ids{0};
    const uint64_t this_build = same_rest_launch ? ++build_ids : 0;
    hipEvent_t t0 = b->lean ? nullptr : b->ev0, t_mid = b->lean ? nullptr : (bb.reg ? b->ev0 : b->ev_mid), t1 = b->lean ? nullptr : b->ev1;
    for (int i = 0; i < b->n; ++i) note_build_enqueued(b->ctxs[i], b->ev1, stream, b, t0, t_mid, t1, &bb, this_build);
    if (shared_qnn)
        for (int i = 0; i < b->n; ++i) b->ctxs[i]->have_factor = false;
    arm_status(b->ctxs, b->n, stream, bb.reg != 0, b->ev1, b->status_ev);
    return FD_OK;
}

static int batch_poll(fd_batch *b)
{
    if (b->h_mismatch && *b->h_mismatch != 0) {
        batch_err(b, "shared-rig evaluation: context %d was built on other rest points than context 0 (same address, other "
                     "contents); its frame was passed through", *b->h_mismatch - 1);
        return FD_E_INVALID;
    }
    bool any = false;
    for (int i = 0; i < b->n; ++i) any = any || b->ctxs[i]->status_inflight || b->ctxs[i]->sticky_rc != FD_OK;
    if (!any) return FD_OK;
    bool shared_pending = false;
    hipEvent_t shared_ev = nullptr;
    for (int i = 0; i < b->n; ++i)
        if (b->ctxs[i]->status_inflight && (b->ctxs[i]->status_poll == b->status_ev || b->ctxs[i]->status_poll == b->ev1)) {
            shared_pending = true; shared_ev = b->ctxs[i]->status_poll;
        }
    if (shared_pending) {
        const hipError_t q = hipEventQuery(shared_ev);
        if (q == hipErrorNotReady) { (void)hipGetLastError(); return FD_OK; }
    }
    for (int i = 0; i < b->n; ++i) {
        const bool lu_before = b->ctxs[i]->prefer_lu;
        const int rc = poll_status(b->ctxs[i]);
        if (b->ctxs[i]->prefer_lu != lu_before) b->prepared = false;
        if (rc) { batch_err(b, "context %d: %s", i, b->ctxs[i]->err); return rc; }
    }
    return FD_OK;
}

int fd_batch_build_result(fd_batch *b, fd_report *reports)
{
    if (!b) return FD_E_INVALID;
    int first = FD_OK;
    for (int i = 0; i < b->n; ++i) {
        const int rc = fd_build_result(b->ctxs[i], reports ? &reports[i] : nullptr);
        if (rc && !first) { first = rc; batch_err(b, "context %d: %s", i, b->ctxs[i]->err); }
    }
    return first;
}

int fd_solve_operator(fd_ctx *ctx, double *S)
{
    if (!ctx || !S) return FD_E_INVALID;
    if (!ctx->points_set) { set_err(ctx, "fd_solve_operator: no control points (call fd_set_points first)"); return FD_E_NOT_BUILT; }
    int rc = use_device(ctx);
    if (rc) return rc;
    FD_HIP(ctx, hipStreamSynchronize(cur_stream(ctx)));
    const int M = ctx->M, rows = model_centres(ctx) + 4;
    const int builds = (M + 2) / 3;
    const int nh = builds < kMaxBatch ? builds : kMaxBatch;
    fd_ctx *helpers[kMaxBatch] = {};
    DevBuf<float> d_unit;
    fd_batch *batch = nullptr;
    auto done = [&](int code) {
        if (batch) fd_batch_destroy(batch);
        for (fd_ctx *h : helpers) if (h) fd_destroy(h);
        d_unit.reset();
        return code;
    };
    fd_config cfg{};
    cfg.struct_size = (int)sizeof(cfg);
    cfg.device = ctx->device; cfg.eval_precision = ctx->eval_precision; cfg.solver = ctx->solver;
    for (int i = 0; i < nh; ++i) {
        fd_ctx *h = helpers[i] = fd_create(&cfg);
        if (!h) { set_err(ctx, "fd_solve_operator: %s", g_err); return done(FD_E_NOMEM); }
        if ((rc = fd_set_kernel(h, ctx->kind, ctx->params, ctx->nparams)) || (rc = fd_set_term(h, ctx->term))) {
            set_err(ctx, "fd_solve_operator: %s", h->err);
            return done(rc);
        }
        h->prefer_lu = ctx->prefer_lu;
        h->stream_ = cur_stream(ctx);
    }
    const size_t per = (size_t)M * 3;
    if (d_unit.alloc(per * (size_t)nh) != hipSuccess) {
        (void)hipGetLastError();
        set_err(ctx, "fd_solve_operator: hipMalloc(%zu bytes) failed", sizeof(float) * per * (size_t)nh);
        return done(FD_E_NOMEM);
    }
    std::vector<float> unit(per * (size_t)nh);
    std::vector<double> W((size_t)rows * 3);
// ... 316 lines not shown
    sc.consumed = true;
    sc.eval_pending = record_eval(sc.eval_ev, stream);
}

static void shot_vectors_evaluated(ShotScratch &sc, hipStream_t stream)
{
    if (sc.eval_pending && hipEventRecord(sc.eval_ev, stream) == hipSuccess) return;
    (void)hipGetLastError();
    (void)hipStreamSynchronize(stream);
}

static bool one_build(const fd_batch *b)
{
    const uint64_t id = b->ctxs[0]->rig_build_id;
    if (id == 0) return false;
    for (int i = 1; i < b->n; ++i)
        if (b->ctxs[i]->rig_build_id != id) return false;
    return true;
}

static int vectors_per_context(fd_batch *b, hipStream_t stream, int precision, hipEvent_t consumed_ev, int64_t N, const float *d_P_in,
                               float *const *d_P_out, const float *d_dist2, float *const *d_falloff_out, const float *d_tu,
                               const float *d_tv, const float *d_nrm, float radius2, float falloffrate, const fd_batch_vectors *vec)
{
    for (int i = 0; i < b->n; ++i) {
        DeformArgs a = deform_args(b->ctxs[i], Mesh{N, d_P_in, d_dist2, d_tu, d_tv, d_nrm, radius2, falloffrate}, d_P_out[i],
                                   d_falloff_out ? d_falloff_out[i] : nullptr);
        a.precision = precision;
        const VectorArgs v{vec->N, vec->tu, vec->tv, vec->N ? vec->N_out[i] : nullptr, vec->tu ? vec->tu_out[i] : nullptr,
                           vec->tv ? vec->tv_out[i] : nullptr, vec->jacobian ? vec->jacobian[i] : nullptr};
        hipError_t e = launch_vectors(a, v, stream);
        if (e != hipSuccess) { batch_err(b, "launch_vectors failed: %s", hipGetErrorString(e)); return FD_E_DEVICE; }
    }
    if (hipEventRecord(consumed_ev, stream) != hipSuccess) { (void)hipGetLastError(); return FD_E_DEVICE; }
    return FD_OK;
}

static int shared_pack(fd_batch *b, hipStream_t stream, int ek, float *const *d_P_out, float *const *d_falloff_out)
{
    fd_ctx *c0 = b->ctxs[0];
    const int si = b->packed_valid ? (b->cur_set ^ 1) : 0;
    fd_batch::SharedSet &st = b->sets[si];
    SharedDeformArgs a{};
    a.N = 1; a.Mpad = round_up(c0->M, kRecPad); a.nF = b->n; a.kind = ek; a.ctiles = c0->d_tiles16;
    a.falloff_out = d_falloff_out;
    int rc;
    if (!b->lean && (rc = batch_poll(b))) return rc;
    for (int i = 0; i < b->n; ++i) {
        fd_ctx *c = b->ctxs[i];
        a.rec32[i] = c->d_rec32; a.model[i] = c->d_model; a.P_out[i] = d_P_out[i]; a.centres[i] = c->d_centres;
        if ((rc = order_after_batch(c, stream))) { batch_err(b, "context %d: %s", i, c->err); return rc; }
    }
    if (one_build(b)) for (int i = 1; i < b->n; ++i) a.centres[i] = a.centres[0];
    const SharedPlan pl = shared_plan(a.Mpad, a.nF, a.kind);
    const size_t wb = pl.wtile_bytes, fb = pl.frame_bytes;
    if (wb > st.d_wtiles.cap || fb > st.d_frames.cap) {
        st.d_wtiles.reset(); st.d_frames.reset(); st.eval_pending = false;
        if (st.d_wtiles.grow(wb) != hipSuccess || st.d_frames.grow(fb) != hipSuccess) {
            (void)hipGetLastError();
            batch_err(b, "shared-rig evaluation: scratch allocation (%zu bytes) failed", wb + fb);
            return FD_E_NOMEM;
        }
    }
    if ((rc = wait_last_eval(b, "shared-rig evaluation", stream, &st.eval_pending, st.eval_done))) return rc;
    a.wtiles = st.d_wtiles; a.frames = st.d_frames;
    a.packed_ev = b->lean ? nullptr : (st.packed_ev.make() ? st.packed_ev : nullptr);
    b->consumed_override = nullptr;
    a.mode = 1;
    a.M = c0->M;
    if (b->h_mismatch && hipHostGetDevicePointer((void **)&a.mismatch, b->h_mismatch, 0) != hipSuccess) { (void)hipGetLastError(); a.mismatch = nullptr; }
    hipError_t e = launch_deform_shared(a, stream);
    if (e != hipSuccess) { batch_err(b, "launch_deform_shared (pack) failed: %s", hipGetErrorString(e)); return FD_E_DEVICE; }
    b->cur_set = si;
    b->packed_valid = b->lean || st.packed_ev != nullptr;
    b->prepared = true;
    for (int i = 0; i < b->n; ++i) {
        b->prep_P_out[i] = d_P_out[i]; b->prep_fall[i] = d_falloff_out ? d_falloff_out[i] : nullptr;
        b->prep_gen[i] = b->ctxs[i]->model_gen;
    }
    b->prep_has_fall = d_falloff_out != nullptr;
    return FD_OK;
}

int fd_batch_prepare_shared(fd_batch *b, void *hip_stream, float *const *d_P_out, float *const *d_falloff_out)
{
    if (!b || !d_P_out) return FD_E_INVALID;
    fd_ctx *c0 = b->ctxs[0];
    int rc = use_device(c0);
    if (rc) { batch_err(b, "%s", c0->err); return rc; }
    hipStream_t stream = hip_stream ? (hipStream_t)hip_stream : cur_stream(c0);
    int ek = 0;
    const int applies = shared_applies(b, "fd_batch_prepare_shared", d_P_out, &ek);
    if (applies < 0) return applies;
    if (applies == 0) return FD_OK;
    return shared_pack(b, stream, ek, d_P_out, d_falloff_out);
}

int fd_batch_deform_shared_dev(fd_batch *b, void *hip_stream, int64_t N, const float *d_P_in, float *const *d_P_out,
                               const float *d_dist2, float *const *d_falloff_out, const float *d_tu,
                               const float *d_tv, const float *d_nrm, float radius2, float falloffrate)
{
    if (!b || !d_P_out) return FD_E_INVALID;
    int rc = shot_check_mesh(b, "fd_batch_deform_shared_dev", N, d_P_in, d_tu, d_tv, d_nrm);
    if (rc) return rc;
    if (N == 0) return FD_OK;
    fd_ctx *c0 = b->ctxs[0];
    rc = use_device(c0);
    if (rc) { batch_err(b, "%s", c0->err); return rc; }
    hipStream_t stream = hip_stream ? (hipStream_t)hip_stream : cur_stream(c0);
    int ek = 0;
    const int applies = shared_applies(b, "fd_batch_deform_shared_dev", d_P_out, &ek);
    if (applies < 0) return applies;
    if (applies == 0) {
        const float *pin[kMaxBatch], *pd2[kMaxBatch], *ptu[kMaxBatch], *ptv[kMaxBatch], *pnr[kMaxBatch];
        for (int i = 0; i < b->n; ++i) { pin[i] = d_P_in; pd2[i] = d_dist2; ptu[i] = d_tu; ptv[i] = d_tv; pnr[i] = d_nrm; }
        rc = fd_batch_deform_dev(b, hip_stream, N, pin, d_P_out, d_dist2 ? pd2 : nullptr, d_falloff_out, d_tu ? ptu : nullptr,
                                 d_tu ? ptv : nullptr, d_tu ? pnr : nullptr, radius2, falloffrate);
        if (rc == FD_OK && b->fallback_ev.make()) {
            if (hipEventRecord(b->fallback_ev, stream) != hipSuccess) { (void)hipGetLastError(); rc = FD_E_DEVICE; }
            b->packed_valid = false;
            b->consumed_override = nullptr;
        }
        return rc;
    }
    bool reuse = b->prepared && b->prep_has_fall == (d_falloff_out != nullptr);
    for (int i = 0; reuse && i < b->n; ++i)
        reuse = b->prep_P_out[i] == d_P_out[i] && (!d_falloff_out || b->prep_fall[i] == d_falloff_out[i]) &&
                b->prep_gen[i] == b->ctxs[i]->model_gen;
    if (reuse) {
        if (!b->lean && (rc = batch_poll(b))) return rc;
        if (!b->prepared) reuse = false;
        for (int i = 0; reuse && i < b->n; ++i)
            if ((rc = order_after_batch(b->ctxs[i], stream))) { batch_err(b, "context %d: %s", i, b->ctxs[i]->err); return rc; }
    }
    if (reuse) {
        fd_batch::SharedSet &ps = b->sets[b->cur_set];
        if (!b->lean && ps.packed_ev && hipStreamWaitEvent(stream, ps.packed_ev, 0) != hipSuccess) {
            batch_err(b, "fd_batch_deform_shared_dev: hipStreamWaitEvent failed: %s", hipGetErrorString(hipGetLastError()));
            return FD_E_DEVICE;
        }
    } else if ((rc = shared_pack(b, stream, ek, d_P_out, d_falloff_out))) {
        return rc;
    }
    fd_batch::SharedSet &st = b->sets[b->cur_set];
    SharedDeformArgs a{};
    a.N = N; a.P_in = d_P_in; a.dist2 = d_dist2; a.tu = d_tu; a.tv = d_tv; a.nrm = d_nrm;
    a.radius2 = radius2; a.falloffrate = falloffrate;
    a.Mpad = round_up(c0->M, kRecPad); a.nF = b->n;
    a.ctiles = c0->d_tiles16;
    a.kind = ek;
    a.falloff_out = d_falloff_out;
    for (int i = 0; i < b->n; ++i) { a.rec32[i] = b->ctxs[i]->d_rec32; a.model[i] = b->ctxs[i]->d_model; a.P_out[i] = d_P_out[i]; }
    a.wtiles = st.d_wtiles; a.frames = st.d_frames;
    a.packed_ev = nullptr;
    a.mode = 2;
    a.delta_out = c0->output == FD_OUTPUT_DISPLACEMENT;
    a.max_wgs = b->eval_cus;
    hipError_t e = launch_deform_shared(a, stream);
    if (e != hipSuccess) { batch_err(b, "launch_deform_shared failed: %s", hipGetErrorString(e)); return FD_E_DEVICE; }
    if (b->lean) {
        st.eval_done = b->ev1;
        st.eval_pending = true;
    } else {
        st.eval_pending = record_eval(st.eval_ev, stream);
        st.eval_done = st.eval_ev;
    }
// ... 397 lines not shown
    if (b->n < shared_vectors_ml64_min_frames(ml_layers(c0))) {
        return vectors_per_context(b, stream, FD_EVAL_FP64, b->sml64.consumed_ev, N, d_P_in, d_P_out, d_dist2, d_falloff_out, d_tu, d_tv, d_nrm,
                                   radius2, falloffrate, vec);
    }
    SharedVectorMl64Args a{};
    fill_mesh(a, N, d_P_in, d_dist2, d_tu, d_tv, d_nrm, radius2, falloffrate);
    a.M = c0->M; a.layers = ml_layers(c0); a.nF = b->n;
    fill_vector_tables(a, b->n, vec);
    a.scratch = b->sml64.d;
    a.max_wgs = b->eval_cus;
    hipError_t e = launch_vectors_shared_ml64(a, stream);
    if (e != hipSuccess) { batch_err(b, "launch_vectors_shared_ml64 failed: %s", hipGetErrorString(e)); return FD_E_DEVICE; }
    shot_vectors_evaluated(b->sml64, stream);
    return FD_OK;
}

const char *fd_shared_vectors_ml_fp64_kernel_name(int M, int layers, int frames)
{
    return shared_vectors_ml64_kernel_name(M, layers, frames);
}

int fd_batch_wait_consumed(fd_batch *b, void *hip_stream)
{
    if (!b) return FD_E_INVALID;
    hipEvent_t ev = b->consumed_override ? b->consumed_override : (b->packed_valid ? b->sets[b->cur_set].packed_ev : b->fallback_ev);
    hipEvent_t evs[5] = {ev, nullptr, nullptr, nullptr, nullptr};
    int n_ev = ev ? 1 : 0;
    for (const ShotScratch *sc : {&b->s64, &b->sml, &b->sml64, &b->sadjp})
        if (sc->consumed) evs[n_ev++] = sc->consumed_ev;
    if (n_ev == 0) return FD_OK;
    fd_ctx *c0 = b->ctxs[0];
    int rc = use_device(c0);
    if (rc) { batch_err(b, "%s", c0->err); return rc; }
    hipStream_t stream = hip_stream ? (hipStream_t)hip_stream : cur_stream(c0);
    for (int i = 0; i < n_ev; ++i)
        if (hipStreamWaitEvent(stream, evs[i], 0) != hipSuccess) {
            batch_err(b, "fd_batch_wait_consumed: hipStreamWaitEvent failed: %s", hipGetErrorString(hipGetLastError()));
            return FD_E_DEVICE;
        }
    return FD_OK;
}

int fd_batch_cook_group(fd_batch *b, void *build_stream, void *eval_stream, const float *d_rest_xyz,
                        const float *const *d_delta_xyz, int M, int64_t N, const float *d_P_in, float *const *d_P_out,
                        float *const *d_falloff_out, const fd_group_events *events)
{
    if (!b || !d_rest_xyz || !d_delta_xyz || !d_P_out) return FD_E_INVALID;
    fd_ctx *c0 = b->ctxs[0];
    hipStream_t bs = build_stream ? (hipStream_t)build_stream : cur_stream(c0);
    hipStream_t es = eval_stream ? (hipStream_t)eval_stream : bs;
    auto mark = [&](void *ev, hipStream_t st) { if (ev && hipEventRecord((hipEvent_t)ev, st) != hipSuccess) (void)hipGetLastError(); };
#ifdef FD_TUNING
    static const bool cook_timing = tuning_env("FD_COOK_TIMING") != nullptr;
    struct CookClock {
        bool on; double t[6]; int n = 0;
        static double now() { timespec ts; clock_gettime(CLOCK_MONOTONIC, &ts); return ts.tv_sec * 1e6 + ts.tv_nsec * 1e-3; }
        void tick() { if (on && n < 6) t[n++] = now(); }
        ~CookClock() { if (on && n == 6) fprintf(stderr, "[cook_group host us] wait_consumed %.1f | set_points %.1f | build %.1f | packing %.1f | evaluation %.1f\n", t[1] - t[0], t[2] - t[1], t[3] - t[2], t[4] - t[3], t[5] - t[4]); }
    } clk{cook_timing};
#define FD_COOK_TICK() clk.tick()
#else
#define FD_COOK_TICK()
#endif
    FD_COOK_TICK();
    int rc = fd_batch_wait_consumed(b, build_stream);
    if (rc) return rc;
    FD_COOK_TICK();
    const float *rest[kMaxBatch];
    for (int i = 0; i < b->n; ++i) rest[i] = d_rest_xyz;
    if ((rc = fd_batch_set_points_dev(b, rest, d_delta_xyz, M))) return rc;
    const bool lean = es == bs;
    struct LeanScope {
        fd_batch *b; hipStream_t s; bool on, built = false;
        ~LeanScope() {
            if (!on) return;
            if (built && hipEventRecord(b->ev1, s) != hipSuccess) (void)hipGetLastError();
            b->prepared = false;
            b->lean = false;
        }
    } scope{b, bs, lean};
    b->lean = lean;
    FD_COOK_TICK();
    if (events) mark(events->before_build, bs);
    if ((rc = fd_batch_build_async(b, build_stream))) return rc;
    scope.built = true;
    if (events) mark(events->after_build, bs);
    FD_COOK_TICK();
    if ((rc = fd_batch_prepare_shared(b, build_stream, d_P_out, d_falloff_out))) return rc;
    FD_COOK_TICK();
    if (es != bs) {
        if (!b->group_ev.make() || hipEventRecord(b->group_ev, bs) != hipSuccess || hipStreamWaitEvent(es, b->group_ev, 0) != hipSuccess) {
            batch_err(b, "fd_batch_cook_group: ordering the evaluation stream failed: %s", hipGetErrorString(hipGetLastError()));
            return FD_E_DEVICE;
        }
    }
    if (events) mark(events->before_eval, es);
    rc = fd_batch_deform_shared_dev(b, es, N, d_P_in, d_P_out, nullptr, d_falloff_out, nullptr, nullptr, nullptr, 1.0f, 1.0f);
    if (events) mark(events->after_eval, es);
    FD_COOK_TICK();
    if (lean && rc == FD_OK && b->packed_valid && b->sets[b->cur_set].eval_pending) b->consumed_override = b->ev1;
    return rc;
}

int fd_batch_set_eval_cus(fd_batch *b, int n_cus)
{
    if (!b) return FD_E_INVALID;
    b->eval_cus = n_cus > 0 ? n_cus : 0;
    return FD_OK;
}

int fd_batch_set_shared_factor(fd_batch *b, int on)
{
    if (!b) return FD_E_INVALID;
    b->shared_factor = on ? 1 : 0;
    return FD_OK;
}

int fd_batch_last_build_shared_factor(const fd_batch *b) { return b ? b->last_shared_factor : 0; }

const char *fd_shared_ml_build_kernel_name(int M, int layers, int frames) { return ml_shared_kernel_name(M, layers, frames); }

int fd_batch_set_shared_lu(fd_batch *b, int on)
{
    if (!b) return FD_E_INVALID;
    b->shared_lu = on ? 1 : 0;
    return FD_OK;
}

const char *fd_shared_qnn_build_kernel_name(int M, int frames) { return qnn_shared_kernel_name(M, frames); }

int fd_batch_size(const fd_batch *b) { return b ? b->n : 0; }

const char *fd_shared_kernel_name(int M, int frames, int kind)
{
    const bool takes = (kind == FD_KERNEL_THIN_PLATE || kind == FD_KERNEL_GAUSSIAN || kind == FD_KERNEL_GAUSSIAN_QNN) && M > 0 && round_up(M, kRecPad) >= 32 &&
                       frames >= 1 && frames <= kMaxBatch;
    return takes ? shared_plan(round_up(M, kRecPad), frames, kind).kernel : "";
}

}

#include "fd_shot_dev.h"

struct fd_shot_dev {
    fd_ctx *engine = nullptr;
    Stream work, copy;
    DevBuf<float> d_rig;
    int M = 0, F = 0;
    DevBuf<float> d_vecs;
    const float *v_in[3] = {nullptr, nullptr, nullptr};
    struct Set {
        DevBuf<float> d;
        Event eval_ev, delivered_ev;
        bool delivering = false;
    } sets[2];
    int set_frames = 0;
    int64_t set_Np = 0;
    bool set_fall = false;
    int set_nvec = 0;
    char err[512] = {0};
};

static void shot_err(fd_shot_dev *sd, const char *fmt, ...)
{
    va_list ap;
    va_start(ap, fmt);
    vsnprintf(sd->err, sizeof(sd->err), fmt, ap);
    va_end(ap);
}

static int shot_failed(fd_shot_dev *sd, const char *call, hipError_t e)
// ... 272 lines not shown
```

### facedeform_amd/csrc/fd_eval_shared.hip

```cpp
#include <cstdio>
#include <cstdlib>

#include <type_traits>

#include "fd_eval_common.h"
#include "fd_shared_common.h"
#include "fd_shared_plan.h"

namespace fd {

namespace {


static_assert(sizeof(MfmaTileH) == kMfmaTileHBytes && sizeof(SharedFrame) == kSharedFrameBytes, "fd_shared_plan.h is sized by these");

struct SharedOut {
    float *P_out[kMaxBatch];
    float *falloff_out[kMaxBatch];
};

struct SharedParams {
    int64_t N;
    const float *P_in;
    const float *dist2;
    const float *tu, *tv, *nrm;
    float radius2, falloffrate;
    int ntiles;
    int nkb;
    int nF, nT;
    int kchunk;
    const MfmaTileH *ctiles;
    const float *norm;
    const uint4 *wtiles;
    const SharedFrame *frames;
    int fast;
    int delta;
    unsigned long long *stamps;
};

struct SharedSlots {
    const Rec32 *rec32[kMaxBatch];
    const DevModel *model[kMaxBatch];
    const double *centres[kMaxBatch];
    int M;
    int nreal;
    int *mismatch;
};

__device__ __forceinline__ bool rig_matches(const SharedSlots &slots, int f, int nF, int l, int per)
{
    bool same = true;
    if (f > 0 && f < nF && slots.centres[f] != slots.centres[0]) {
        const double *a = slots.centres[f], *b0 = slots.centres[0];
        const int n = 3 * slots.M;
        bool diff = false;
        int e = l;
        for (; e + 7 * per < n; e += 8 * per) {
            double va[8], vb[8];
#pragma unroll
            for (int u = 0; u < 8; ++u) { va[u] = a[e + u * per]; vb[u] = b0[e + u * per]; }
#pragma unroll
            for (int u = 0; u < 8; ++u) diff |= !(va[u] == vb[u]);
        }
        for (; e < n; e += per) diff |= !(a[e] == b0[e]);
        same = !diff;
    }
    for (int off = per / 2; off >= 1; off >>= 1) same = (__shfl_xor((int)same, off) != 0) && same;
    if (!same && l == 0 && slots.mismatch) *slots.mismatch = (f < slots.nreal ? f : slots.nreal - 1) + 1;
    return same;
}

__global__ __launch_bounds__(256) void k_pack_shared(const SharedSlots slots, const SharedOut out, int nF, int Mpad, int dense,
                                                      uint4 *wtiles, SharedFrame *frames, const MfmaTileH *ctiles, int gauss,
                                                      size_t poly_at, size_t copy_at, size_t norm_at)
{
    const int kb = blockIdx.x, T = blockIdx.y, nT = gridDim.y;
    constexpr int per = (int)(sizeof(MfmaTileH) / 16);
    uint4 *copy = wtiles + copy_at;
    if (T == 0 && gauss) {
        if (threadIdx.x < 32) {
            const int centre = 32 * kb + (int)threadIdx.x;
            copy[(size_t)2 * kb * per + threadIdx.x] =
                centre < Mpad ? *reinterpret_cast<const uint4 *>(&slots.rec32[0][centre]) : make_uint4(0u, 0u, 0u, 0u);
        }
    } else if (T == 0) {
        const int ntiles = Mpad / 16;
        if ((int)threadIdx.x < 2 * per) {
            const int tile = 2 * kb + (int)threadIdx.x / per;
            copy[(size_t)2 * kb * per + threadIdx.x] =
// ... 377 lines not shown
                normalize3(u[0], u[1], u[2]);
                normalize3(v[0], v[1], v[2]);
                normalize3(n[0], n[1], n[2]);
                float gm[3][3];
#pragma unroll
                for (int r = 0; r < 3; ++r)
#pragma unroll
                    for (int c = 0; c < 3; ++c) gm[r][c] = u[r] * u[c] + v[r] * v[c] + n[r] * n[c];
#pragma unroll
                for (int c = 0; c < 3; ++c) {
                    a1[c] = u[0] * gm[0][c] + u[1] * gm[1][c] + u[2] * gm[2][c];
                    a2[c] = v[0] * gm[0][c] + v[1] * gm[1][c] + v[2] * gm[2][c];
                }
                normalize3(a1[0], a1[1], a1[2]);
                normalize3(a2[0], a2[1], a2[2]);
            }
        }
#pragma unroll
        for (int fs = 0; fs < kSlots; ++fs) {
            {
                const int f = fs;
                if (f >= p.nF) continue;
                const float inv = __uint_as_float((unsigned)__builtin_amdgcn_readlane((int)tab[(8 * f) / 64], (8 * f) % 64));
                const bool built = __builtin_amdgcn_readlane((int)tab[(8 * f + 1) / 64], (8 * f + 1) % 64) != 0;
                const uint64_t pout = ((uint64_t)(unsigned)__builtin_amdgcn_readlane((int)tab[(8 * f + 5) / 64], (8 * f + 5) % 64) << 32) |
                                      (unsigned)__builtin_amdgcn_readlane((int)tab[(8 * f + 4) / 64], (8 * f + 4) % 64);
                const uint64_t fout = ((uint64_t)(unsigned)__builtin_amdgcn_readlane((int)tab[(8 * f + 7) / 64], (8 * f + 7) % 64) << 32) |
                                      (unsigned)__builtin_amdgcn_readlane((int)tab[(8 * f + 6) / 64], (8 * f + 6) % 64);
                if (!doit) continue;
                Pos3 FD_GLOBAL *dstP = (Pos3 FD_GLOBAL *)((char FD_GLOBAL *)(pout + 12ull * (uint64_t)vbase) + off12);
                if (!built) {
                    if (p.delta) store_pos3(dstP, 0.f, 0.f, 0.f);
                else if (pout != (uint64_t)p.P_in) store_pos3(dstP, pos[0], pos[1], pos[2]);
                    continue;
                }
                float disp[3];
                if constexpr (DENSE) {
                    const int B = fs / 16, k = (fs % 16) / 4, r = fs % 4;
                    disp[0] = acc[3 * B][k][r] * inv; disp[1] = acc[3 * B + 1][k][r] * inv; disp[2] = acc[3 * B + 2][k][r] * inv;
                } else {
                    const int T = fs / 4, k = fs % 4;
                    disp[0] = acc[T][k][0] * inv; disp[1] = acc[T][k][1] * inv; disp[2] = acc[T][k][2] * inv;
                }
                if (p.tu) {
                    const float da1 = disp[0] * a1[0] + disp[1] * a1[1] + disp[2] * a1[2];
                    const float da2 = disp[0] * a2[0] + disp[1] * a2[1] + disp[2] * a2[2];
#pragma unroll
                    for (int c = 0; c < 3; ++c) disp[c] = a1[c] * da1 + a2[c] * da2;
                }
                if (fout) __builtin_nontemporal_store(fall, (float FD_GLOBAL *)((char FD_GLOBAL *)(fout + 4ull * (uint64_t)vbase) + off4));
                store_pos3_nt(dstP, base[0] + disp[0] * fall, base[1] + disp[1] * fall, base[2] + disp[2] * fall);
            }
        }
        FD_SSTAMP(3)
    };
    int grp = blockIdx.x;
    bool built_here = true;
#pragma unroll
    for (int q = 0; q < kTabRegs; ++q) {
        const int idx = 64 * q + lane;
        if (idx < kSlots * 8 && (idx & 7) == 1) built_here = built_here && tab[q] != 0u;
    }
    if (p.fast && __all(built_here)) {
        const int nfull = (int)(p.N / kSharedThreads);
        for (; grp < nfull; grp += gridDim.x) do_group(grp, std::true_type{});
    }
    for (; grp < ngroups; grp += gridDim.x) do_group(grp, std::false_type{});
    if (stamp && lane == 0) {
        for (int q = 0; q < 4; ++q) p.stamps[wave * 8 + q] = st_acc[q];
    }
#undef FD_SSTAMP
}


typedef float f32x16 __attribute__((ext_vector_type(16)));

__global__ __launch_bounds__(256) void k_pack_shared_wide(const SharedSlots slots, const SharedOut out, int nF, int nslot, int Mpad,
                                                           uint4 *wtiles, SharedFrame *frames, const MfmaTileH *ctiles, int gauss, int layout,
                                                           size_t poly_at, size_t copy_at, size_t norm_at)
{
    const int kb = blockIdx.x, T = blockIdx.y, NT = gridDim.y;
    const int w16 = wide_w16(NT);
    if (T == 0) {
        uint2 *dst = reinterpret_cast<uint2 *>(wtiles + copy_at) + (size_t)kb * 128;
        if (gauss) {
            if (threadIdx.x < 32) {
                const int centre = 32 * kb + (int)threadIdx.x;
                wtiles[copy_at + (size_t)kb * 64 + threadIdx.x] =
                    centre < Mpad ? *reinterpret_cast<const uint4 *>(&slots.rec32[0][centre]) : make_uint4(0u, 0u, 0u, 0u);
            }
        } else if (layout == 1) {
            if (threadIdx.x < 64) {
                const int lane = threadIdx.x, h = lane >> 5, r = lane & 31;
                const int tile = 2 * kb + (r >> 4);
                uint4 v = make_uint4(0u, 0u, 0u, 0u);
                if (tile < Mpad / 16) {
                    const unsigned *a0 = ctiles[tile].a[16 * (2 * h) + (r & 15)], *a1 = ctiles[tile].a[16 * (2 * h + 1) + (r & 15)];
                    v = make_uint4(a0[0], a0[1], a1[0], a1[1]);
                }
                wtiles[copy_at + (size_t)kb * 64 + lane] = v;
            }
        } else if (threadIdx.x < 128) {
            const int i = threadIdx.x >> 6, lane = threadIdx.x & 63, h = lane >> 5, r = lane & 31;
            const int tile = 2 * kb + (r >> 4);
            uint2 v = make_uint2(0u, 0u);
            if (tile < Mpad / 16) { const unsigned *a = ctiles[tile].a[16 * (2 * i + h) + (r & 15)]; v = make_uint2(a[0], a[1]); }
            dst[threadIdx.x] = v;
        }
        if (kb == 0 && threadIdx.x == 255) {
            const float *nn = slots.model[0]->norm32;
            wtiles[norm_at] = make_uint4(__float_as_uint(nn[0]), __float_as_uint(nn[1]), __float_as_uint(nn[2]), __float_as_uint(nn[3]));
        }
    }
    __shared__ float s_scale[kWideSlots];
    {
        const int f = threadIdx.x >> 3, l = threadIdx.x & 7;
        float m = 0.f;
        if (f < nslot) {
            m = slots.model[f]->wmax32;
        }
        for (int off = 4; off >= 1; off >>= 1) m = fmaxf(m, __shfl_xor(m, off));
        const bool same_rig = (kb == 0 && T == 0) ? rig_matches(slots, f, nslot, l, 8) : true;
        if (l == 0) {
            int k = 0;
            if (m > 0.f && m < INFINITY) k = 13 - (__builtin_amdgcn_frexp_expf(m) - 1);
            k = k < -100 ? -100 : (k > 100 ? 100 : k);
            s_scale[f] = ldexpf(1.f, k);
            if (kb == 0 && T == 0) {
                SharedFrame fr;
                fr.inv_scale = ldexpf(1.f, -k - (gauss ? kGaussShift : 0));
                fr.built = (f < nslot && same_rig && slots.model[f]->terminationtype == 1) ? 1 : 0;
                fr.pad[0] = fr.pad[1] = 0;
                fr.P_out = f < nslot ? out.P_out[f] : nullptr;
                fr.falloff_out = f < nslot ? out.falloff_out[f] : nullptr;
                frames[f] = fr;
            }
        }
    }
    __syncthreads();
    if (threadIdx.x >= 128) return;
    const int s = threadIdx.x >> 6, lane = threadIdx.x & 63, h = lane >> 5;
    int f, c;
    if (layout == 1) {
        const int rho = lane & 31, k = 16 * T + 4 * (rho >> 3) + (rho & 3);
        f = 2 * (k / 3) + ((rho >> 2) & 1); c = k % 3;
    } else {
        const int row = 32 * T + (lane & 31);
        f = row / 3; c = row % 3;
    }
    const bool live = f < nslot;
    const float sc = live ? s_scale[f] : 0.f;
    f16x8 hi, lo;
#pragma unroll
    for (int m = 0; m < 8; ++m) {
        const int centre = 32 * kb + 8 * (2 * s + (m >> 2)) + 4 * h + (m & 3);
        float w = 0.f;
        if (live && centre < Mpad) {
            const Rec32 r = slots.rec32[f][centre];
            w = (c == 0 ? r.wx : (c == 1 ? r.wy : r.wz)) * sc;
        }
        const _Float16 hh = (_Float16)w;
        hi[m] = hh;
        lo[m] = (_Float16)(w - (float)hh);
    }
    uint4 *dst = wtiles + (size_t)kb * w16 + (size_t)((T * 2 + s) * 2) * 64;
    dst[lane] = __builtin_bit_cast(uint4, hi);
    dst[64 + lane] = __builtin_bit_cast(uint4, lo);
    if (kb == 0 && s == 0) {
        f16x8 pt;
#pragma unroll
        for (int m = 0; m < 8; ++m) {
            const int coef = h == 0 ? (m < 5 ? m : m - 4) : (m == 0 ? 4 : (m < 6 ? m - 1 : -1));
            const bool want_lo = h == 1 && m >= 1;
            float w = 0.f;
            if (live && coef >= 0) w = slots.model[f]->poly32[5 * c + coef] * sc;
            const _Float16 hh = (_Float16)w;
            pt[m] = want_lo ? (_Float16)(w - (float)hh) : hh;
        }
        wtiles[poly_at + (size_t)T * 64 + lane] = __builtin_bit_cast(uint4, pt);
    }
}

constexpr int kWideVpm = 3;
constexpr int kW1Vpm = 3;

template <bool GAUSS, int NT, int NSLOT>
__global__ __launch_bounds__(64 * kWideWaves) __attribute__((amdgpu_waves_per_eu(kWideWaves / 4, kWideWaves / 4)))
void k_deform32_tps_shared_wide(const SharedParams p, int ngroups)
{
    constexpr int WAVES = kWideWaves, THREADS = 64 * WAVES;
    static_assert(NSLOT % 4 == 0 && NSLOT <= kWideSlots && 3 * NSLOT <= 32 * NT, "frame slots in fours, three rows each");
    constexpr int kWideW16 = wide_w16(NT);
    constexpr int TV = 2;
    constexpr int kSlots = kWideSlots;
    extern __shared__ __attribute__((aligned(16))) char smem[];
    SharedFrame *s_frames = reinterpret_cast<SharedFrame *>(smem);
    uint4 *s_poly = reinterpret_cast<uint4 *>(smem + sizeof(SharedFrame) * (size_t)kSlots);
    uint2 *s_ct = reinterpret_cast<uint2 *>(s_poly + NT * 64);
    uint4 *s_w = reinterpret_cast<uint4 *>(s_ct + (size_t)128 * p.kchunk);
    uint64_t *s_ftab = reinterpret_cast<uint64_t *>(s_w + (size_t)kWideW16 * p.kchunk);
    unsigned *s_ticket = reinterpret_cast<unsigned *>(s_ftab + 512);
    const int tid = threadIdx.x;
    const int lane = tid & 63;
    const int wave = __builtin_amdgcn_readfirstlane(tid >> 6);
    const int h = lane >> 5, j = lane & 31;
    const float n0 = p.norm[0], n1 = p.norm[1], n2 = p.norm[2];
    const float inv_s = p.norm[3];
    const bool resident = p.nkb <= p.kchunk;
    const unsigned long long st_t0 = p.stamps ? __builtin_amdgcn_s_memtime() : 0, st_r0 = p.stamps ? __builtin_amdgcn_s_memrealtime() : 0;
    f32x16 zero16;
#pragma unroll
    for (int r = 0; r < 16; ++r) zero16[r] = 0.f;

    auto stage = [&](int kb0, int nk) {
        __syncthreads();
        {
            const uint4 *src = reinterpret_cast<const uint4 *>(p.ctiles) + (size_t)kb0 * 64;
            uint4 *dst = reinterpret_cast<uint4 *>(s_ct);
            for (int q = tid; q < nk * 64; q += THREADS) dst[q] = src[q];
        }
        {
            const u32x4 *src = reinterpret_cast<const u32x4 *>(p.wtiles + (size_t)kb0 * kWideW16);
            u32x4 *dst = reinterpret_cast<u32x4 *>(s_w);
            const int n16 = nk * kWideW16;
            int q = tid;
            for (; q + 7 * THREADS < n16; q += 8 * THREADS) {
                const u32x4 v0 = src[q], v1 = src[q + THREADS], v2 = src[q + 2 * THREADS], v3 = src[q + 3 * THREADS];
                const u32x4 v4 = src[q + 4 * THREADS], v5 = src[q + 5 * THREADS], v6 = src[q + 6 * THREADS], v7 = src[q + 7 * THREADS];
                dst[q] = v0; dst[q + THREADS] = v1; dst[q + 2 * THREADS] = v2; dst[q + 3 * THREADS] = v3;
                dst[q + 4 * THREADS] = v4; dst[q + 5 * THREADS] = v5; dst[q + 6 * THREADS] = v6; dst[q + 7 * THREADS] = v7;
            }
            for (; q < n16; q += THREADS) dst[q] = src[q];
        }
        __syncthreads();
    };

    constexpr int kTabRegs = (kSlots * 8 + 63) / 64;
    unsigned tab[kTabRegs];
#pragma unroll
    for (int q = 0; q < kTabRegs; ++q) tab[q] = reinterpret_cast<const unsigned *>(p.frames)[64 * q + lane];
    {
        const uint4 *src = reinterpret_cast<const uint4 *>(p.frames);
        uint4 *dst = reinterpret_cast<uint4 *>(s_frames);
        for (int q = tid; q < kSlots * (int)(sizeof(SharedFrame) / 16); q += THREADS) dst[q] = src[q];
        const uint4 *psrc = p.wtiles + (size_t)p.nkb * kWideW16;
        for (int q = tid; q < NT * 64; q += THREADS) s_poly[q] = psrc[q];
        if (tid == 0) *s_ticket = 0u;
        __syncthreads();
        if (p.fast && tid < NSLOT * 16) s_ftab[tid] = (uint64_t)p.frames[4 * (tid >> 6) + ((tid & 63) >> 4)].falloff_out + 16u * (unsigned)(tid & 15);
    }
    if (resident) {
        stage(0, p.nkb);
        if (wave >= 4) __builtin_amdgcn_s_sleep(12);
    } else {
        __syncthreads();
    }

    const bool stamp = p.stamps != nullptr && blockIdx.x == 0;
    unsigned long long st_prev = 0, st_acc[5] = {0, 0, 0, 0, 0};
#define FD_SSTAMP(K) if (stamp) { __builtin_amdgcn_sched_barrier(0); const unsigned long long t_ = __builtin_amdgcn_s_memtime(); st_acc[K] += t_ - st_prev; st_prev = t_; __builtin_amdgcn_sched_barrier(0); }
    if (stamp) st_prev = __builtin_amdgcn_s_memtime();
    struct GroupRaw { float p[TV][3]; float d2[TV]; };
    const bool dynamic = resident;
// ... 831 lines not shown
```

### facedeform_amd/csrc/fd_internal.h

```cpp
#pragma once

#include <hip/hip_runtime.h>
#include <stdint.h>

#include "../../include/facedeform_hip.h"

#include "fd_tuning.h"

namespace fd {

#define FD_GLOBAL __attribute__((address_space(1)))
typedef double FD_GLOBAL gdouble;
typedef const double FD_GLOBAL gcdouble;
template <typename T> __host__ __device__ __forceinline__ T FD_GLOBAL *as_global(T *p) { return (T FD_GLOBAL *)p; }

struct Rec32 {
    float cx, cy, cz, s;
    float wx, wy, wz, pad;
};
struct Rec64 {
    double cx, cy, cz, s;
    double wx, wy, wz, pad;
};

// ... 43 lines not shown
static inline int round_up(int v, int m) { return (v + m - 1) / m * m; }

constexpr int kPanelThreads = 1024;
constexpr int kMaxOrder = 5632;
constexpr int kRhsCols = 16;
constexpr int kMovesStride = 132;
static inline int lu_step_capacity(int npad) { return npad / 4 + 2; }

constexpr int kMaxBatch = 32;

struct BatchSlot {
    float *rest, *delta;
    double *centres;
    double *radii;
    double *A;
    double *X;
    double *W;
    int *ipiv;
    int *moves;
    Rec32 *rec32;
    Rec64 *rec64;
    MfmaTile *tiles;
    MfmaTileH *tiles16;
    DevModel *model;
    double *ns;
    int *host_status;
};

inline unsigned device_cus()
{
    static unsigned cached[64] = {};
    int dev = 0;
    if (hipGetDevice(&dev) != hipSuccess) { (void)hipGetLastError(); return 256u; }
    if (dev >= 0 && dev < 64 && cached[dev]) return cached[dev];
    int n = 0;
    if (hipDeviceGetAttribute(&n, hipDeviceAttributeMultiprocessorCount, dev) != hipSuccess || n <= 0) { (void)hipGetLastError(); n = 256; }
    if (dev >= 0 && dev < 64) cached[dev] = (unsigned)n;
    return (unsigned)n;
}

struct PointSrc {
    const float *rest[kMaxBatch];
    const float *delta[kMaxBatch];
};

struct BuildBuffers {
    int M, T, n, npad, lda, ncols;
    int kind, term;
    double lambda;
    double gauss_R, qnn_q, qnn_z;
    int Mpad;
    const BatchSlot *d_slots;
    int nbatch;
    int group_panels;
    int small;
    int reg;
    int reg_front;
    int spd;
    int nopivot;
    int ml_layers;
};

hipError_t launch_prepare(const BuildBuffers &b, hipStream_t stream, const PointSrc *src);
hipError_t launch_build(const BuildBuffers &b, hipStream_t stream, hipEvent_t ev_mid);
hipError_t launch_resolve(const BuildBuffers &b, hipStream_t stream, const PointSrc *src);
hipError_t launch_pack(const BuildBuffers &b, hipStream_t stream);
hipError_t launch_pack_from_weights(const BuildBuffers &b, hipStream_t stream, int layers = 0);
hipError_t launch_assemble_block(const BuildBuffers &b, hipStream_t stream, int npad_a, int radii_off = 0);
hipError_t launch_pack_records(const BuildBuffers &b, hipStream_t stream, int records, int kind, int mode, int layers);
hipError_t launch_backsub_rows(const BuildBuffers &b, hipStream_t stream, int rows);
hipError_t launch_prepare_rhs(const BuildBuffers &b, hipStream_t stream, const PointSrc *src);
hipError_t launch_backsub_update(const BuildBuffers &b, hipStream_t stream, int row_lo, int w);
hipError_t launch_qnn_radii(const BuildBuffers &b, hipStream_t stream);
hipError_t launch_lu_factor_solve(const BuildBuffers &b, hipStream_t stream);
hipError_t launch_lu_factor(const BuildBuffers &b, hipStream_t stream);
hipError_t launch_lu_resolve_core(const BuildBuffers &b, hipStream_t stream);

bool spd_applicable(int kind, int term, double lambda, int M);
bool small_applicable(int M, int T);
static inline size_t ns_doubles(int M) { return (size_t)12 * (size_t)M + 64 + (size_t)(M / 32 + 2) * 66 * 32; }
hipError_t launch_build_spd(const BuildBuffers &b, hipStream_t stream, hipEvent_t ev_mid);
hipError_t launch_resolve_spd(const BuildBuffers &b, hipStream_t stream, const PointSrc *src);
bool reg_applicable(int kind, int term, double lambda, int M);
hipError_t launch_build_reg(const BuildBuffers &b, hipStream_t stream, const PointSrc *src, hipEvent_t ev_mid);
hipError_t launch_build_reg_shared(const BuildBuffers &b, hipStream_t stream, const PointSrc *src, hipEvent_t ev_mid, double *fac);
size_t reg_factor_doubles();
hipError_t reg_build_init();
constexpr int kMaxLayers = 8;
hipError_t launch_build_ml(const BuildBuffers &b, hipStream_t stream, hipEvent_t ev_mid);
bool ml_shared_applies(int M, int layers, int frames);
int ml_shared_min_frames();
const char *ml_shared_kernel_name(int M, int layers, int frames);
hipError_t ml_shared_init();
size_t ml_shared_scratch_bytes(const BuildBuffers &b);
const BatchSlot *ml_shared_slots(void *scratch);
hipError_t launch_build_ml_shared(const BuildBuffers &b, hipStream_t stream, void *scratch);
struct MlSharedLayout { int tau, R, aff, ld, ld_stride, ld_inv; };
hipError_t launch_ml_shared_init(const BuildBuffers &b, hipStream_t stream, void *scratch);
hipError_t launch_ml_solve_shared(const BuildBuffers &b, hipStream_t stream, void *scratch, const MlSharedLayout &at);
bool qnn_shared_applies(int M, int frames);
int qnn_shared_min_frames();
const char *qnn_shared_kernel_name(int M, int frames);
hipError_t qnn_shared_init();
size_t qnn_shared_scratch_bytes(const BuildBuffers &b);
const BatchSlot *qnn_shared_slot(void *scratch);
hipError_t launch_build_qnn_shared(const BuildBuffers &b, hipStream_t stream, void *scratch, bool fill_slot);
hipError_t launch_qnn_shared_init(const BuildBuffers &b, hipStream_t stream, void *scratch);
hipError_t launch_qnn_solve_shared(const BuildBuffers &b, hipStream_t stream, void *scratch, const MlSharedLayout &at);
hipError_t launch_build_qnn(const BuildBuffers &b, hipStream_t stream, hipEvent_t ev_mid);
hipError_t launch_resolve_qnn(const BuildBuffers &b, hipStream_t stream, const PointSrc *src);

struct DeformArgs {
    int64_t N;
    const float *P_in; float *P_out;
    const float *dist2; float *falloff_out;
    const float *tu, *tv, *nrm;
    float radius2, falloffrate;
    int M, Mpad, kind;
    const Rec32 *rec32; const Rec64 *rec64;
    const MfmaTile *tiles;
    const MfmaTileH *tiles16;
    const DevModel *model;
    int precision, variant;
    int layers;
    int delta_out;
};
hipError_t launch_deform(const DeformArgs &a, hipStream_t stream);
struct VectorArgs {
    const float *N, *tu, *tv;
    float *N_out, *tu_out, *tv_out;
    float *jacobian;
};
hipError_t launch_vectors(const DeformArgs &a, const VectorArgs &v, hipStream_t stream);
constexpr int kInvertDefaultIter = 20, kInvertMaxIter = 64;
struct InvertArgs {
    int max_iter;
    double tol;
    float *residual_out;
    int *iters_out;
};
hipError_t launch_invert(const DeformArgs &a, const InvertArgs &v, hipStream_t stream);
struct AdjointArgs {
    const float *G;
    double *grad_W;
    double *partial;
    int T;
};
int adjoint_groups(int64_t N);
hipError_t launch_adjoint(const DeformArgs &a, const AdjointArgs &g, hipStream_t stream);
struct AdjointPointsArgs {
    const float *G;
    double *grad_P;
    double *grad_f;
};
hipError_t launch_adjoint_points(const DeformArgs &a, const AdjointPointsArgs &g, hipStream_t stream);
struct AdjointShotArgs {
    const float *G;
    double *grad_W;
    double *partial;
    int F, T;
};
int adjoint_shot_ranges(int64_t N, int C);
size_t adjoint_shot_partial_doubles(int64_t N, int C);
hipError_t launch_adjoint_shot(const DeformArgs &a, const AdjointShotArgs &g, hipStream_t stream);
struct GramArgs {
    const float *omega;
    double *H;
// ... 138 lines not shown
```

### facedeform_amd/csrc/fd_pack.h

```cpp
#pragma once

#include "fd_internal.h"

namespace fd {
namespace packing {

__device__ __forceinline__ double block_sum(double v, double *scratch, int tid)
{
    for (int off = 32; off >= 1; off >>= 1) v += __shfl_xor(v, off);
    __syncthreads();
    if ((tid & 63) == 0) scratch[tid >> 6] = v;
    __syncthreads();
    return scratch[0] + scratch[1] + scratch[2] + scratch[3];
}
__device__ __forceinline__ double block_max(double v, double *scratch, int tid)
{
    for (int off = 32; off >= 1; off >>= 1) { const double o = __shfl_xor(v, off); v = o > v ? o : v; }
    __syncthreads();
    if ((tid & 63) == 0) scratch[tid >> 6] = v;
    __syncthreads();
    const double a = scratch[0] > scratch[1] ? scratch[0] : scratch[1];
    const double b = scratch[2] > scratch[3] ? scratch[2] : scratch[3];
    return a > b ? a : b;
}
// ... 11 lines not shown
    if ((tid & 63) == 0) {
#pragma unroll
        for (int q = 0; q < N; ++q) scratch[(tid >> 6) * N + q] = v[q];
    }
    __syncthreads();
#pragma unroll
    for (int q = 0; q < N; ++q) {
        if (MAX) {
            const double a = scratch[q] > scratch[N + q] ? scratch[q] : scratch[N + q];
            const double b = scratch[2 * N + q] > scratch[3 * N + q] ? scratch[2 * N + q] : scratch[3 * N + q];
            v[q] = a > b ? a : b;
        } else {
            v[q] = scratch[q] + scratch[N + q] + scratch[2 * N + q] + scratch[3 * N + q];
        }
    }
}

struct PackGlobal {
    const double *X, *W, *centres, *radii;
    const float *dl;
    const DevModel *model;
    int npad, from_w;
    __device__ __forceinline__ double centre(int j, int q) const { return centres[3 * j + q]; }
    __device__ __forceinline__ bool has_delta() const { return dl != nullptr; }
    __device__ __forceinline__ double delta(int j, int q) const { return (double)dl[3 * j + q]; }
    __device__ __forceinline__ double weight(int j, int c) const { return from_w ? W[3 * j + c] : X[(size_t)c * npad + j]; }
    __device__ __forceinline__ double affine(int cc, int k, int M, int T) const
    {
        if (from_w) return W[3 * (M + k) + cc];
        return k < T ? X[(size_t)cc * npad + M + k] : 0.0;
    }
    __device__ __forceinline__ double radius(int j) const { return radii[j]; }
    __device__ __forceinline__ int sing_flag() const { return model->sing_flag; }
    __device__ __forceinline__ int dup_flag() const { return model->dup_flag; }
};

constexpr float kTpsGradLog2e = 1.4426950408889634f;
__host__ __device__ constexpr double grad_scale64(int kind)
{
    return kind == FD_KERNEL_BIHARMONIC ? 1.0 : (kind == FD_KERNEL_CUBIC ? 3.0 : 2.0);
}
__host__ __device__ constexpr float grad_scale32(int kind)
{
    return kind == FD_KERNEL_GAUSSIAN || kind == FD_KERNEL_GAUSSIAN_QNN ? (float)(2.0 * 0.6931471805599453)
                                                                        : (float)grad_scale64(kind);
}
template <int KIND>
__device__ __forceinline__ double grad64(double d2, double s)
{
    if constexpr (KIND == FD_KERNEL_THIN_PLATE) {
        return d2 > 0.0 ? log(d2) + 1.0 : 0.0;
    } else if constexpr (KIND == FD_KERNEL_GAUSSIAN || KIND == FD_KERNEL_GAUSSIAN_QNN) {
        return exp(d2 * s) * s;
    } else if constexpr (KIND == FD_KERNEL_BIHARMONIC) {
        return d2 > 0.0 ? 1.0 / sqrt(d2) : 0.0;
    } else {
        return sqrt(d2);
    }
}

template <int KIND>
__device__ __forceinline__ void phi_grad64(double d2, double s, double &phi, double &g)
{
    if constexpr (KIND == FD_KERNEL_THIN_PLATE) {
        const double l = d2 > 0.0 ? log(d2) : 0.0;
        phi = d2 * l;
        g = d2 > 0.0 ? l + 1.0 : 0.0;
    } else if constexpr (KIND == FD_KERNEL_GAUSSIAN || KIND == FD_KERNEL_GAUSSIAN_QNN) {
        phi = exp(d2 * s);
        g = phi * s;
    } else if constexpr (KIND == FD_KERNEL_BIHARMONIC) {
        phi = sqrt(d2);
        g = d2 > 0.0 ? 1.0 / phi : 0.0;
    } else {
        g = sqrt(d2);
        phi = d2 * g;
    }
}
__host__ __device__ constexpr double weight_scale64(int kind)
{
    return kind == FD_KERNEL_THIN_PLATE ? 0.5 : (kind == FD_KERNEL_BIHARMONIC ? -1.0 : 1.0);
}

template <class Src>
__device__ __forceinline__ void pack_body_from(const Src &in, const BatchSlot &slot, int , int M, int Mpad, int T, int kind, int from_w, int layers)
{
    double *W = slot.W;
    Rec32 *rec32 = slot.rec32;
    Rec64 *rec64 = slot.rec64;
    DevModel *model = slot.model;
    __shared__ int s_bad;
    __shared__ double s_red[4 * 18];
    const int tid = threadIdx.x;
    if (tid == 0) s_bad = 0;
    __syncthreads();
    const double kLn2 = 0.6931471805599453;
    const double kLog2e = 1.4426950408889634;
    const bool gauss = kind == FD_KERNEL_GAUSSIAN || kind == FD_KERNEL_GAUSSIAN_QNN;

    double sx = 0.0, sy = 0.0, sz = 0.0;
    for (int j = tid; j < M; j += 256) { sx += in.centre(j, 0); sy += in.centre(j, 1); sz += in.centre(j, 2); }
    double csum[3] = {sx, sy, sz};
    block_reduce_many<3, false>(csum, s_red, tid);
    double cenx = csum[0] / M, ceny = csum[1] / M, cenz = csum[2] / M;
    double r2 = 0.0, r2o = 0.0;
    const bool dl = in.has_delta();
    double dmax2 = 0.0, ndmin2 = -INFINITY;
    for (int j = tid; j < M; j += 256) {
        const double x = in.centre(j, 0), y = in.centre(j, 1), z = in.centre(j, 2);
        const double d = (x - cenx) * (x - cenx) + (y - ceny) * (y - ceny) + (z - cenz) * (z - cenz);
        r2 = d > r2 ? d : r2;
        const double o = x * x + y * y + z * z;
        r2o = o > r2o ? o : r2o;
        if (dl) {
            const double a = in.delta(j, 0), b = in.delta(j, 1), c2 = in.delta(j, 2);
            const double dd = a * a + b * b + c2 * c2;
            dmax2 = dd > dmax2 ? dd : dmax2;
            ndmin2 = -dd > ndmin2 ? -dd : ndmin2;
        }
    }
    double ext[4] = {r2, r2o, dmax2, ndmin2};
    block_reduce_many<4, true>(ext, s_red, tid);
    if (dl) {
        const double moving2 = 1e-2 * ext[2];
        double nmin[1] = {-INFINITY};
        for (int j = tid; j < M; j += 256) {
            const double a = in.delta(j, 0), b = in.delta(j, 1), c2 = in.delta(j, 2);
            const double dd = a * a + b * b + c2 * c2;
            if (dd >= moving2 && dd > 0.0 && -dd > nmin[0]) nmin[0] = -dd;
        }
        block_reduce_many<1, true>(nmin, s_red, tid);
        ext[3] = nmin[0] > -INFINITY ? nmin[0] : 0.0;
    }
    const double rad_c = sqrt(ext[0]);
    const double rad_o = sqrt(ext[1]);
    const double cen = sqrt(cenx * cenx + ceny * ceny + cenz * cenz);
    double x0[3] = {0.0, 0.0, 0.0};
    double rad = rad_o;
    if (cen > rad_c * 0.0625) { x0[0] = (double)(float)cenx; x0[1] = (double)(float)ceny; x0[2] = (double)(float)cenz; rad = rad_c; }
    double sc = 1.0;
    if (rad > 0.0 && isfinite(rad)) {
        int e = (int)rint(log2(rad));
        e = e < -100 ? -100 : (e > 100 ? 100 : e);
        sc = ldexp(1.0, e);
    }
    const double inv_s = 1.0 / sc;
    double w32 = 1.0, w64 = 1.0, kappa = 0.0;
    if (kind == FD_KERNEL_THIN_PLATE) { w32 = 0.5 * kLn2 * sc * sc; w64 = 0.5; kappa = sc * sc * log(sc); }
    if (kind == FD_KERNEL_BIHARMONIC) { w32 = -sc; w64 = -1.0; }
    if (kind == FD_KERNEL_CUBIC) { w32 = sc * sc * sc; }

    bool bad = false;
    float wmax = 0.f;
    double m[18];
#pragma unroll
    for (int q = 0; q < 18; ++q) m[q] = 0.0;
    for (int j = tid; j < Mpad; j += 256) {
        Rec32 r32 = {0.f, 0.f, 0.f, 0.f, 0.f, 0.f, 0.f, 0.f};
        Rec64 r64 = {0.0, 0.0, 0.0, 0.0, 0.0, 0.0, 0.0, 0.0};
        if (j < M) {
            const double w[3] = {in.weight(j, 0), in.weight(j, 1), in.weight(j, 2)};
            bad |= !(isfinite(w[0]) && isfinite(w[1]) && isfinite(w[2]));
            if (!from_w) { W[3 * j] = w[0]; W[3 * j + 1] = w[1]; W[3 * j + 2] = w[2]; }
            const double R = in.radius(j);
            r64.cx = in.centre(j, 0); r64.cy = in.centre(j, 1); r64.cz = in.centre(j, 2);
            r64.s = gauss ? -1.0 / (R * R) : 0.0;
            r64.wx = w[0] * w64; r64.wy = w[1] * w64; r64.wz = w[2] * w64;
            const double cn[3] = {(r64.cx - x0[0]) * inv_s, (r64.cy - x0[1]) * inv_s, (r64.cz - x0[2]) * inv_s};
            r32.cx = (float)cn[0]; r32.cy = (float)cn[1]; r32.cz = (float)cn[2];
            r32.s = gauss ? (float)(-kLog2e * sc * sc / (R * R)) : 0.f;
            r32.wx = (float)(w[0] * w32); r32.wy = (float)(w[1] * w32); r32.wz = (float)(w[2] * w32);
            wmax = fmaxf(wmax, fmaxf(fabsf(r32.wx), fmaxf(fabsf(r32.wy), fabsf(r32.wz))));
            const double cc2 = cn[0] * cn[0] + cn[1] * cn[1] + cn[2] * cn[2];
#pragma unroll
            for (int c = 0; c < 3; ++c) {
                m[5 * c] += w[c];
                m[5 * c + 1] += w[c] * cn[0];
                m[5 * c + 2] += w[c] * cn[1];
                m[5 * c + 3] += w[c] * cn[2];
                m[5 * c + 4] += w[c] * cc2;
                m[15 + c] += fabs(w[c] * w32);
            }
        }
        int jo = j;
        if (layers > 1 && j < M) { const int Mc = M / layers; jo = (j % Mc) * layers + j / Mc; }
        rec32[jo] = r32;
        rec64[jo] = r64;
    }
    block_reduce_many<18, false>(m, s_red, tid);
    double wm[1] = {(double)wmax};
    block_reduce_many<1, true>(wm, s_red, tid);

    __shared__ double s_aff[12];
    if (tid < 12) {
        const int cc = tid / 4, k = tid % 4;
        const double v = in.affine(cc, k, M, T);
        bad |= !isfinite(v);
        if (!from_w) W[3 * (M + k) + cc] = v;
        model->affine64[tid] = v;
        s_aff[tid] = v;
    }
    if (bad) s_bad = 1;
    __syncthreads();
    float pmax = 0.f;
    if (tid < 3) {
        const int c = tid;
        const double *a = s_aff + 4 * c;
        const float p5[5] = {(float)(a[0] + a[1] * x0[0] + a[2] * x0[1] + a[3] * x0[2] + kappa * m[5 * c + 4]),
                             (float)(a[1] * sc - 2.0 * kappa * m[5 * c + 1]), (float)(a[2] * sc - 2.0 * kappa * m[5 * c + 2]),
                             (float)(a[3] * sc - 2.0 * kappa * m[5 * c + 3]), (float)(kappa * m[5 * c])};
#pragma unroll
        for (int e = 0; e < 5; ++e) { model->poly32[5 * c + e] = p5[e]; pmax = fmaxf(pmax, fabsf(p5[e])); }
        model->norm32[c] = (float)x0[c];
    }
    pmax = fmaxf(pmax, fmaxf(__shfl(pmax, 1), __shfl(pmax, 2)));
    if (tid == 0) {
        model->wmax32 = fmaxf((float)wm[0], pmax);
        const double phimax = kind == FD_KERNEL_THIN_PLATE ? 8.0 : (kind == FD_KERNEL_CUBIC ? 8.0 : (kind == FD_KERNEL_BIHARMONIC ? 2.0 : 1.0));
        double S = 0.0;
#pragma unroll
        for (int c = 0; c < 3; ++c) {
            const double *a = s_aff + 4 * c;
            const double poly = fabs(a[0]) + (fabs(a[1]) + fabs(a[2]) + fabs(a[3])) * (rad_o > 0.0 ? rad_o : 1.0) + 4.0 * fabs(kappa * m[5 * c]);
            const double v = m[15 + c] * phimax + poly;
            S = v > S ? v : S;
        }
        const double dmax = sqrt(ext[2]), dmin = dl ? sqrt(-ext[3]) : 0.0;
        model->fp32_error = S * 2.98023223876953125e-08;
        model->cancellation = dmax > 0.0 ? S / dmax : 0.0;
        model->delta_min = dmin;
        model->delta_max = dmax;
        model->extent = rad_o;
        model->norm32[3] = (float)inv_s;
        int tt = 1;
        if (from_w == 1) {
            if (s_bad) tt = -4;
        } else {
            if (in.sing_flag() || s_bad) tt = -4;
            if (in.dup_flag()) tt = -5;
        }
        model->terminationtype = tt;
        if (slot.host_status) *slot.host_status = tt;
    }
}

__device__ __forceinline__ void pack_body(const BatchSlot &slot, int npad, int M, int Mpad, int T, int kind, int from_w, int layers)
{
    const PackGlobal in{from_w ? nullptr : slot.X, slot.W, slot.centres, slot.radii, from_w ? nullptr : slot.delta, slot.model, npad, from_w};
    pack_body_from(in, slot, npad, M, Mpad, T, kind, from_w, layers);
}

__device__ __forceinline__ void split3_bf16(float x, unsigned &hi, unsigned &mid, unsigned &lo)
{
    const unsigned u = __float_as_uint(x);
    const float r1 = x - __uint_as_float(u & 0xffff0000u);
    const unsigned u1 = __float_as_uint(r1);
    const float r2 = r1 - __uint_as_float(u1 & 0xffff0000u);
    hi = u >> 16; mid = u1 >> 16; lo = __float_as_uint(r2) >> 16;
}

__device__ __forceinline__ void pack_tiles_body(const BatchSlot &slot, int Mpad, int tile, int lane)
{
    const Rec32 *rec32 = slot.rec32;
    MfmaTile *tiles = slot.tiles;
    const int g = lane >> 4, i = lane & 15;
    const Rec32 r = rec32[16 * tile + i];
    unsigned h, m, l;
    unsigned k[8] = {0, 0, 0, 0, 0, 0, 0, 0};
    if (g < 3) {
        const float c = g == 0 ? r.cx : (g == 1 ? r.cy : r.cz);
        split3_bf16(c, h, m, l);
        k[0] = h; k[1] = h; k[2] = m; k[3] = m; k[4] = h; k[5] = l;
    } else {
        const float cc = fmaf(r.cz, r.cz, fmaf(r.cy, r.cy, r.cx * r.cx));
        split3_bf16(cc, h, m, l);
        k[0] = h; k[1] = m; k[2] = l;
        k[3] = 0x3f80; k[4] = 0x3f80; k[5] = 0x3f80;
    }
    MfmaTile &t = tiles[tile];
    t.a[lane][0] = k[0] | (k[1] << 16);
    t.a[lane][1] = k[2] | (k[3] << 16);
    t.a[lane][2] = k[4] | (k[5] << 16);
    t.a[lane][3] = k[6] | (k[7] << 16);
    if (i < 12) {
        const int pair = i / 6, c = (i % 6) / 2, half = i % 2;
        const Rec32 rw = rec32[16 * tile + 4 * g + 2 * pair + half];
        t.w[g][i] = c == 0 ? rw.wx : (c == 1 ? rw.wy : rw.wz);
    }
    if (lane < 16) t.pad[lane] = 0.f;
    (void)Mpad;

    MfmaTileH *tiles16 = slot.tiles16;
    if (tiles16) {
        MfmaTileH &th = tiles16[tile];
        const float v = g < 3 ? (g == 0 ? r.cx : (g == 1 ? r.cy : r.cz)) : fmaf(r.cz, r.cz, fmaf(r.cy, r.cy, r.cx * r.cx));
        const _Float16 vh = (_Float16)v;
        const _Float16 vl = (_Float16)(v - (float)vh);
        const unsigned uh = (unsigned)__builtin_bit_cast(unsigned short, vh), ul = (unsigned)__builtin_bit_cast(unsigned short, vl);
        if (g < 3) { th.a[lane][0] = uh | (uh << 16); th.a[lane][1] = ul | (ul << 16); }
        else { th.a[lane][0] = uh | (ul << 16); th.a[lane][1] = 0x3c003c00u; }
        if (i < 12) th.w[g][i] = t.w[g][i];
        if (lane < 16) th.pad[lane] = 0.f;
    }
}

}
}
```

Measured before the change: 56800.

## Split packing tail into separate kernel, precompute normalisation, fold wide-tile packing

Moves the centre/delta normalisation reduction into an extra block of k_reg_front2, so it runs in parallel with the factorisation tiles, and stores it in the front buffer. The packing stage leaves the non-front k_build_reg and runs in a new 256-thread k_reg_tail kernel that builds records and the model in LDS and copies them out. For thin-plate batches this kernel can also write the shared wide fp16 weight, poly and centre tiles directly, which removes a later separate packing pass. This adds a kernel launch and more code paths that must keep the model layout consistent.

```diff
diff --git a/facedeform_amd/_build.py b/facedeform_amd/_build.py
--- a/facedeform_amd/_build.py
+++ b/facedeform_amd/_build.py
@@ -18,7 +18,7 @@
                "fd_adjoint_shot.hip": ["-mllvm", "-disable-machine-licm"],
                "fd_adjoint_points.hip": ["-mllvm", "-disable-machine-licm"],
                "fd_adjoint_points_shot.hip": ["-mllvm", "-disable-machine-licm"]}
-HEADERS = [os.path.join(CSRC, "fd_internal.h"), os.path.join(CSRC, "fd_tuning.h"), os.path.join(CSRC, "fd_pack.h"), os.path.join(CSRC, "fd_eval_common.h"), os.path.join(CSRC, "fd_transport.h"), os.path.join(CSRC, "fd_eval_point.h"), os.path.join(CSRC, "fd_shot_launch.h"), os.path.join(CSRC, "fd_vectors_shot.h"), os.path.join(CSRC, "fd_shared64.h"), os.path.join(CSRC, "fd_shared_ml64.h"), os.path.join(CSRC, "fd_shared_ml.h"), os.path.join(CSRC, "fd_shared_common.h"), os.path.join(CSRC, "fd_shared_plan.h"), os.path.join(CSRC, "fd_shared_solve.h"), os.path.join(CSRC, "fd_shot_dev.h"), os.path.join(CSRC, "fd_fit_host.h"), os.path.join(CSRC, "fd_owned.h"), os.path.join(CSRC, "fd_operator.h"), os.path.join(CSRC, "fd_adjoint_points_shot.h"), os.path.join(CSRC, "fd_bake_plan.h"), os.path.join(_ROOT, "include", "facedeform_hip.h")]
+HEADERS = [os.path.join(CSRC, "fd_internal.h"), os.path.join(CSRC, "fd_tuning.h"), os.path.join(CSRC, "fd_pack.h"), os.path.join(CSRC, "fd_eval_common.h"), os.path.join(CSRC, "fd_transport.h"), os.path.join(CSRC, "fd_eval_point.h"), os.path.join(CSRC, "fd_shot_launch.h"), os.path.join(CSRC, "fd_vectors_shot.h"), os.path.join(CSRC, "fd_shared64.h"), os.path.join(CSRC, "fd_shared_ml64.h"), os.path.join(CSRC, "fd_shared_ml.h"), os.path.join(CSRC, "fd_shared_common.h"), os.path.join(CSRC, "fd_shared_pack.h"), os.path.join(CSRC, "fd_shared_plan.h"), os.path.join(CSRC, "fd_shared_solve.h"), os.path.join(CSRC, "fd_shot_dev.h"), os.path.join(CSRC, "fd_fit_host.h"), os.path.join(CSRC, "fd_owned.h"), os.path.join(CSRC, "fd_operator.h"), os.path.join(CSRC, "fd_adjoint_points_shot.h"), os.path.join(CSRC, "fd_bake_plan.h"), os.path.join(_ROOT, "include", "facedeform_hip.h")]
 
 
 def hipcc_path() -> str:
diff --git a/facedeform_amd/csrc/fd_build_reg.hip b/facedeform_amd/csrc/fd_build_reg.hip
--- a/facedeform_amd/csrc/fd_build_reg.hip
+++ b/facedeform_amd/csrc/fd_build_reg.hip
@@ -1,8 +1,10 @@
+#include <cstddef>
 #include <cstdio>
 #include <cstdlib>
 
 #include "fd_internal.h"
 #include "fd_pack.h"
+#include "fd_shared_pack.h"
 
 namespace fd {
 
@@ -214,13 +216,13 @@
 
 constexpr int kAff = 64;
 struct PackLds {
-    const double *cen, *dlt, *sol, *aff;
+    const double *cen, *sol, *aff;
     const float *dl_global;
     double R;
     int sing, dup;
     __device__ __forceinline__ double centre(int j, int q) const { return cen[3 * j + q]; }
     __device__ __forceinline__ bool has_delta() const { return true; }
-    __device__ __forceinline__ double delta(int j, int q) const { return dlt ? dlt[3 * j + q] : (double)dl_global[3 * j + q]; }
+    __device__ __forceinline__ double delta(int j, int q) const { return (double)dl_global[3 * j + q]; }
     __device__ __forceinline__ double weight(int j, int c) const { return sol[c * 256 + j]; }
     __device__ __forceinline__ double affine(int cc, int k, int, int T) const { return k < T ? aff[3 * k + cc] : 0.0; }
     __device__ __forceinline__ double radius(int) const { return R; }
@@ -488,7 +490,8 @@
 constexpr int kFront1Tiles = kWorkers;
 constexpr int kFront2Tiles = kRegWaves;
 constexpr size_t kFrV = 0, kFrF = 4 * kRows, kFrB21 = 7 * kRows, kFrSmall = 11 * kRows, kFrMeta = kFrSmall + kSmallDoubles,
-                 kFrTile = kFrMeta + 8, kFrY = kFrTile + 2 * (size_t)(kMaxBlocks * (kMaxBlocks + 1) / 2);
+                 kFrTile = kFrMeta + 8, kFrNorm = kFrTile + 2 * (size_t)(kMaxBlocks * (kMaxBlocks + 1) / 2), kFrY = kFrNorm + 16;
+static_assert(packing::kPackNormDoubles <= 16, "the front buffer's room for PackNorm");
 __host__ __device__ inline size_t reg_front_doubles(int M)
 {
     const int nbk = (M + 15) / 16;
@@ -618,7 +621,7 @@
     }
 }
 
-__global__ __launch_bounds__(kRegThreads) void k_reg_front2(const BatchSlot *tab, int M, int T, int tpw)
+__global__ __launch_bounds__(kRegThreads) void k_reg_front2(const BatchSlot *tab, int M, int T, int kind, int tpw)
 {
     const BatchSlot &slot = tab[blockIdx.z];
     __shared__ __attribute__((aligned(16))) double s_mem[8 * kRows + kSmallDoubles];
@@ -630,6 +633,18 @@
     const int n1 = M - T;
     const int nbk = (M + 15) / 16, ntiles = nbk * (nbk + 1) / 2;
     gdouble *fr = as_global(slot.ns);
+    if (blockIdx.x + 1 == gridDim.x) {
+        if (tid >= 256) return;
+        __shared__ double s_red[packing::kPackRedDoubles];
+        const packing::PackGlobal in{nullptr, nullptr, slot.centres, slot.radii, slot.delta, slot.model, 0, 0};
+        const packing::PackNorm nm = packing::pack_normalise(in, M, kind, s_red);
+        if (tid == 0) {
+            const double v[packing::kPackNormDoubles] = {nm.x0[0], nm.x0[1], nm.x0[2], nm.sc, nm.inv_s, nm.w32, nm.w64, nm.kappa, nm.rad_o, nm.dmax, nm.dmin};
+#pragma unroll
+            for (int q = 0; q < packing::kPackNormDoubles; ++q) fr[kFrNorm + q] = v[q];
+        }
+        return;
+    }
     for (int x = tid; x < 4 * kRows; x += kRegThreads) {
         L.V[x] = fr[kFrV + x];
         const int i = x >> 2, t = x & 3, r = i >> 4, row = i & 15;
@@ -737,7 +752,7 @@
     if constexpr (!FRONT) {
         gcdouble *fr = as_global(slot.ns);
         static_assert(4 * kRows == 2 * kRegThreads, "two entries per thread");
-        double lv[2], lb[2], lf[2], ls[2], lc[2], ld[2];
+        double lv[2], lb[2], lf[2], ls[2];
 #pragma unroll
         for (int h = 0; h < 2; ++h) {
             const int e = tid + kRegThreads * h;
@@ -745,8 +760,6 @@
             lb[h] = fr[kFrB21 + e];
             lf[h] = fr[kFrF + (e < 3 * kRows ? e : 0)];
             ls[h] = fr[kFrSmall + (e < kSmallDoubles ? e : 0)];
-            lc[h] = slot.centres[e < 3 * M ? e : 0];
-            ld[h] = (double)slot.delta[e < 3 * M ? e : 0];
         }
 #pragma unroll
         for (int h = 0; h < 2; ++h) {
@@ -755,7 +768,6 @@
             L.B21[e] = lb[h];
             if (e < 3 * kRows) L.F[e] = lf[h];
             if (e < kSmallDoubles) L.small[e] = ls[h];
-            if (e < 3 * M) { L.cen[e] = lc[h]; L.scr[e] = ld[h]; }
         }
     } else {
         const float *rest = use_src ? src.rest[blockIdx.z] : slot.rest;
@@ -1230,9 +1242,9 @@
         for (int q = 0; q < 4; ++q) {
             const int i = lane + 64 * q;
             if (i < M) { X[i] = xr[q][0]; X[(size_t)npad + i] = xr[q][1]; X[2 * (size_t)npad + i] = xr[q][2]; }
-            if (i < M) { L.Y[i] = xr[q][0]; L.Y[256 + i] = xr[q][1]; L.Y[512 + i] = xr[q][2]; }
-        }
-        if (lane < 12) {
+            if (FRONT && i < M) { L.Y[i] = xr[q][0]; L.Y[256 + i] = xr[q][1]; L.Y[512 + i] = xr[q][2]; }
+        }
+        if (FRONT && lane < 12) {
             double v = 0.0;
 #pragma unroll
             for (int k = 0; k < 4; ++k)
@@ -1253,20 +1265,23 @@
             model->terminationtype = 0;
             model->dup_flag = dup_any ? 1 : 0;
             model->sing_flag = (L.stat[2] != 0.0 || L.stat[3] != 0.0) ? 1 : 0;
-            L.stat[4] = (L.stat[2] != 0.0 || L.stat[3] != 0.0) ? 1.0 : 0.0;
-            L.stat[5] = dup_any ? 1.0 : 0.0;
+            if (FRONT) {
+                L.stat[4] = (L.stat[2] != 0.0 || L.stat[3] != 0.0) ? 1.0 : 0.0;
+                L.stat[5] = dup_any ? 1.0 : 0.0;
+            }
             model->iterations = M + T;
             model->amax_bits = (unsigned long long)__double_as_longlong(amax);
             model->pivmin_bits = (unsigned long long)__double_as_longlong(L.stat[0]);
             model->pivmax_bits = (unsigned long long)__double_as_longlong(L.stat[1]);
         }
     }
+    if constexpr (FRONT) {
     __threadfence_block();
     __syncthreads();
     FD_RSTAMP()
     if (tid >= 256) return;
     {
-        const PackLds in{L.cen, FRONT ? nullptr : L.scr, L.Y, L.small + kAff, slot.delta, gauss_R, L.stat[4] != 0.0 ? 1 : 0, L.stat[5] != 0.0 ? 1 : 0};
+        const PackLds in{L.cen, L.Y, L.small + kAff, slot.delta, gauss_R, L.stat[4] != 0.0 ? 1 : 0, L.stat[5] != 0.0 ? 1 : 0};
         packing::pack_body_from(in, slot, npad, M, Mpad, T, kind, 0, 0);
     }
     FD_RSTAMP()
@@ -1275,10 +1290,124 @@
         for (int tile = tid >> 6; tile < Mpad / 16; tile += 4) packing::pack_tiles_body(slot, Mpad, tile, lane);
     }
     FD_RSTAMP()
+    } else {
+        FD_RSTAMP()
+    }
 #undef FD_RSTAMP
 #undef tI
 #undef tJ
 #undef FD_SLOT
+}
+
+struct PackPre {
+    double w[3], cen[3], R, aff;
+    int sing, dup;
+    __device__ __forceinline__ double centre(int, int q) const { return cen[q]; }
+    __device__ __forceinline__ double weight(int, int c) const { return w[c]; }
+    __device__ __forceinline__ double affine(int, int, int, int) const { return aff; }
+    __device__ __forceinline__ double radius(int) const { return R; }
+    __device__ __forceinline__ int sing_flag() const { return sing; }
+    __device__ __forceinline__ int dup_flag() const { return dup; }
+};
+static_assert(16 * kMaxBlocks == 256, "k_reg_tail: one record per thread");
+constexpr int kModelWords = (int)(sizeof(DevModel) / 4), kModelPackedFrom = (int)(offsetof(DevModel, affine64) / 4);
+static_assert(sizeof(DevModel) % 4 == 0 && offsetof(DevModel, terminationtype) == 0 && offsetof(DevModel, affine64) % 4 == 0,
+              "k_reg_tail copies out what the packing writes of a model: its first word and everything from affine64 on");
+
+template <bool FOLD>
+__global__ __launch_bounds__(256) void k_reg_tail(const BatchSlot *tab, int M, int T, int npad, int kind, int Mpad, const TailShared sh)
+{
+    const BatchSlot &slot = tab[blockIdx.z];
+    __shared__ int s_bad;
+    __shared__ double s_red[packing::kPackRedDoubles];
+    __shared__ __attribute__((aligned(16))) Rec32 s_rec[256];
+    __shared__ __attribute__((aligned(16))) unsigned s_model[kModelWords];
+    __shared__ __attribute__((aligned(16))) MfmaTileH s_t16[FOLD ? kMaxBlocks : 1];
+    const int tid = threadIdx.x, lane = tid & 63;
+    packing::PackNorm nm;
+    PackPre in;
+    {
+        gcdouble *fr = as_global(slot.ns) + kFrNorm;
+        gcdouble *X = as_global(slot.X), *cen = as_global(slot.centres);
+        const DevModel FD_GLOBAL *gm = as_global(slot.model);
+        const int j = tid < M ? tid : 0;
+        nm.x0[0] = fr[0]; nm.x0[1] = fr[1]; nm.x0[2] = fr[2];
+        nm.sc = fr[3]; nm.inv_s = fr[4]; nm.w32 = fr[5]; nm.w64 = fr[6]; nm.kappa = fr[7]; nm.rad_o = fr[8]; nm.dmax = fr[9]; nm.dmin = fr[10];
+#pragma unroll
+        for (int q = 0; q < 3; ++q) { in.w[q] = X[(size_t)q * npad + j]; in.cen[q] = cen[3 * j + q]; }
+        in.R = as_global(slot.radii)[j];
+        const int cc = tid < 12 ? tid / 4 : 0, k = tid & 3;
+        const double a = X[(size_t)cc * npad + M + (k < T ? k : 0)];
+        in.aff = (tid < 12 && k < T) ? a : 0.0;
+        in.sing = gm->sing_flag; in.dup = gm->dup_flag;
+    }
+    if (tid == 0) s_bad = 0;
+    if (tid < kModelWords) s_model[tid] = 0u;
+    __syncthreads();
+    BatchSlot ls = slot;
+    ls.rec32 = s_rec;
+    ls.model = reinterpret_cast<DevModel *>(s_model);
+    if (FOLD) ls.tiles16 = s_t16;
+    packing::pack_records(in, nm, ls, M, Mpad, T, kind, 0, 0, &s_bad, s_red);
+    __syncthreads();
+    {
+        const uint4 *src = reinterpret_cast<const uint4 *>(s_rec);
+        uint4 *dst = reinterpret_cast<uint4 *>(slot.rec32);
+        for (int i = tid; i < 2 * Mpad; i += 256) dst[i] = src[i];
+        unsigned FD_GLOBAL *gm = as_global(reinterpret_cast<unsigned *>(slot.model));
+        if (tid < kModelWords && (tid == 0 || tid >= kModelPackedFrom)) gm[tid] = s_model[tid];
+    }
+    if (kind == FD_KERNEL_THIN_PLATE) {
+        for (int tile = tid >> 6; tile < Mpad / 16; tile += 4) packing::pack_tiles_body(ls, Mpad, tile, lane);
+    }
+    if constexpr (FOLD) {
+        const int me = (int)blockIdx.z, nF = sh.nF;
+        const bool last = me == nF - 1;
+        uint4 *wtiles = reinterpret_cast<uint4 *>(sh.wtiles);
+        const DevModel *model = ls.model;
+        const int k = wide_scale_exp(model->wmax32);
+        const float sc = ldexpf(1.f, k);
+        if (tid < kWideSlots && (tid == me || (last && tid > me))) {
+            const bool live = tid < sh.nslot;
+            SharedFrame fr;
+            fr.inv_scale = live ? ldexpf(1.f, -k) : 1.f;
+            fr.built = (live && model->terminationtype == 1) ? 1 : 0;
+            fr.pad[0] = fr.pad[1] = 0;
+            fr.P_out = live ? sh.P_out[me] : nullptr;
+            fr.falloff_out = live ? sh.falloff_out[me] : nullptr;
+            reinterpret_cast<SharedFrame *>(sh.frames)[tid] = fr;
+        }
+        const int w16 = wide_w16(sh.ntiles);
+        for (int it = tid; it < sh.nkb * sh.ntiles * 128; it += 256) {
+            const int ln = it & 63, s = (it >> 6) & 1, Tt = (it >> 7) % sh.ntiles, kb = (it >> 7) / sh.ntiles;
+            int f, c;
+            wide_row(1, Tt, ln & 31, f, c);
+            if ((f < nF ? f : nF - 1) != me) continue;
+            const bool live = f < sh.nslot;
+            wide_pack_weights(wtiles, w16, kb, Tt, s, ln, s_rec, c, live, live ? sc : 0.f, Mpad);
+        }
+        for (int it = tid; it < sh.ntiles * 64; it += 256) {
+            const int ln = it & 63, Tt = it >> 6;
+            int f, c;
+            wide_row(1, Tt, ln & 31, f, c);
+            if ((f < nF ? f : nF - 1) != me) continue;
+            const bool live = f < sh.nslot;
+            wide_pack_poly(wtiles, sh.poly_at, Tt, ln, model->poly32, c, live, live ? sc : 0.f);
+        }
+        __syncthreads();
+        {
+            const uint4 *src = reinterpret_cast<const uint4 *>(s_t16);
+            uint4 *dst = reinterpret_cast<uint4 *>(slot.tiles16);
+            for (int i = tid; i < (Mpad / 16) * (int)(sizeof(MfmaTileH) / 16); i += 256) dst[i] = src[i];
+        }
+        if (me == 0) {
+            for (int it = tid; it < sh.nkb * 128; it += 256) wide_pack_centres(wtiles, sh.copy_at, it >> 7, it & 127, s_t16, Mpad, 1);
+            if (tid == 255) {
+                const float *nn = model->norm32;
+                wtiles[sh.norm_at] = make_uint4(__float_as_uint(nn[0]), __float_as_uint(nn[1]), __float_as_uint(nn[2]), __float_as_uint(nn[3]));
+            }
+        }
+    }
 }
 
 __global__ __launch_bounds__(256) void k_resolve_reg(const BatchSlot *tab, const PointSrc src, int use_src, int M, int T, int npad, int kind,
@@ -1518,9 +1647,10 @@
     return hipGetLastError();
 }
 
-hipError_t launch_build_reg(const BuildBuffers &b, hipStream_t stream, const PointSrc *src, hipEvent_t ev_mid)
+hipError_t launch_build_reg(const BuildBuffers &b, hipStream_t stream, const PointSrc *src, hipEvent_t ev_mid, const TailShared *fold, bool *folded)
 {
     static const PointSrc none{};
+    if (folded) *folded = false;
     const unsigned nbatch = (unsigned)b.nbatch;
     if (ev_mid) (void)hipEventRecord(ev_mid, stream);
     const size_t lds = sizeof(double) * reg_lds_doubles(b.M);
@@ -1542,10 +1672,17 @@
         const int tpw1 = tiles_per_wave(kFront1Tiles), tpw2 = tiles_per_wave(kFront2Tiles);
         hipLaunchKernelGGL(k_reg_front1, dim3((unsigned)((ntiles + kFront1Tiles * tpw1 - 1) / (kFront1Tiles * tpw1)), 1, nbatch), dim3(kRegThreads), 0, stream,
                            b.d_slots, src ? *src : none, src ? 1 : 0, b.M, b.T, b.kind, b.lambda, b.gauss_R, tpw1);
-        hipLaunchKernelGGL(k_reg_front2, dim3((unsigned)((ntiles + kFront2Tiles * tpw2 - 1) / (kFront2Tiles * tpw2)), 1, nbatch), dim3(kRegThreads), 0, stream,
-                           b.d_slots, b.M, b.T, tpw2);
+        hipLaunchKernelGGL(k_reg_front2, dim3((unsigned)((ntiles + kFront2Tiles * tpw2 - 1) / (kFront2Tiles * tpw2)) + 1, 1, nbatch), dim3(kRegThreads), 0, stream,
+                           b.d_slots, b.M, b.T, b.kind, tpw2);
         hipLaunchKernelGGL(k_build_reg<false>, dim3(1, 1, nbatch), dim3(kRegThreads), lds, stream, b.d_slots, none, 0, b.M, b.T,
                            b.npad, b.kind, b.Mpad, b.lambda, b.gauss_R, want_stamps ? d_stamps : nullptr, (double *)nullptr);
+        if (fold && b.kind == FD_KERNEL_THIN_PLATE && fold->nF == b.nbatch && fold->wtiles && fold->frames) {
+            hipLaunchKernelGGL(k_reg_tail<true>, dim3(1, 1, nbatch), dim3(256), 0, stream, b.d_slots, b.M, b.T, b.npad, b.kind, b.Mpad, *fold);
+            if (folded) *folded = true;
+        } else {
+            static const TailShared no_fold{};
+            hipLaunchKernelGGL(k_reg_tail<false>, dim3(1, 1, nbatch), dim3(256), 0, stream, b.d_slots, b.M, b.T, b.npad, b.kind, b.Mpad, no_fold);
+        }
     } else
     hipLaunchKernelGGL(k_build_reg<true>, dim3(1, 1, nbatch), dim3(kRegThreads), lds, stream, b.d_slots, src ? *src : none, src ? 1 : 0, b.M, b.T,
                        b.npad, b.kind, b.Mpad, b.lambda, b.gauss_R, want_stamps ? d_stamps : nullptr, (double *)nullptr);
diff --git a/facedeform_amd/csrc/fd_capi.hip b/facedeform_amd/csrc/fd_capi.hip
--- a/facedeform_amd/csrc/fd_capi.hip
+++ b/facedeform_amd/csrc/fd_capi.hip
@@ -164,6 +164,8 @@
     Event group_ev;
     bool lean = false;
     hipEvent_t consumed_override = nullptr;
+    float *const *fold_P_out = nullptr;
+    float *const *fold_fall = nullptr;
     char err[512] = {0};
 };
 
@@ -1944,6 +1946,8 @@
     return FD_OK;
 }
 
+static int fold_begin(fd_batch *b, hipStream_t stream, const BuildBuffers &bb, TailShared &t, int *set_out);
+
 int fd_batch_build_async(fd_batch *b, void *hip_stream)
 {
     if (!b) return FD_E_INVALID;
@@ -2021,12 +2025,21 @@
         (void)hipGetLastError(); shared_fac = false;
     }
     b->last_shared_factor = (shared_fac || shared_ml || shared_qnn) ? 1 : 0;
+    TailShared fold{};
+    int fold_set = -1;
+    if (b->lean && b->fold_P_out && bb.reg && bb.reg_front && !shared_fac && same_rest_launch) {
+        const int applies = fold_begin(b, stream, bb, fold, &fold_set);
+        if (applies < 0) return applies;
+        if (applies == 0) fold_set = -1;
+    }
     if (!b->lean) FD_BHIP(hipEventRecord(b->ev0, stream));
     if (shared_fac) {
         FD_BHIP(launch_build_reg_shared(bb, stream, &b->src, nullptr, b->d_fac));
         b->have_src = false;
     } else if (bb.reg) {
-        FD_BHIP(launch_build_reg(bb, stream, b->have_src ? &b->src : nullptr, nullptr));
+        bool folded = false;
+        FD_BHIP(launch_build_reg(bb, stream, b->have_src ? &b->src : nullptr, nullptr, fold_set >= 0 ? &fold : nullptr, &folded));
+        if (!folded) fold_set = -1;
         b->have_src = false;
     } else {
     FD_BHIP(launch_prepare(bb, stream, b->have_src ? &b->src : nullptr));
@@ -2057,6 +2070,17 @@
     if (shared_qnn)
         for (int i = 0; i < b->n; ++i) b->ctxs[i]->have_factor = false;
     arm_status(b->ctxs, b->n, stream, bb.reg != 0, b->ev1, b->status_ev);
+    if (fold_set >= 0) {
+        b->consumed_override = nullptr;
+        b->cur_set = fold_set;
+        b->packed_valid = true;
+        b->prepared = true;
+        for (int i = 0; i < b->n; ++i) {
+            b->prep_P_out[i] = b->fold_P_out[i]; b->prep_fall[i] = b->fold_fall ? b->fold_fall[i] : nullptr;
+            b->prep_gen[i] = b->ctxs[i]->model_gen;
+        }
+        b->prep_has_fall = b->fold_fall != nullptr;
+    }
     return FD_OK;
 }
 
@@ -2539,6 +2563,40 @@
     return FD_OK;
 }
 
+static int fold_begin(fd_batch *b, hipStream_t stream, const BuildBuffers &bb, TailShared &t, int *set_out)
+{
+    fd_ctx *c0 = b->ctxs[0];
+    if (eval_kind(c0) != FD_KERNEL_THIN_PLATE || bb.kind != FD_KERNEL_THIN_PLATE || bb.nbatch != b->n) return 0;
+    for (int i = 0; i < b->n; ++i) {
+        fd_ctx *c = b->ctxs[i];
+        if (!b->fold_P_out[i] || !c->rest_src || c->rest_src != c0->rest_src || c->output != c0->output || !c->d_tiles16 ||
+            c->eval_precision != FD_EVAL_FP32 || c->eval_variant > 0 || record_layers(c) != 0)
+            return 0;
+    }
+    const int Mpad = round_up(c0->M, kRecPad);
+    if (Mpad < 32 || Mpad != bb.Mpad) return 0;
+    const SharedPlan pl = shared_plan(Mpad, b->n, FD_KERNEL_THIN_PLATE);
+    if (pl.variant != 3 || pl.kchunk < 1) return 0;
+    const int si = b->packed_valid ? (b->cur_set ^ 1) : 0;
+    fd_batch::SharedSet &st = b->sets[si];
+    if (pl.wtile_bytes > st.d_wtiles.cap || pl.frame_bytes > st.d_frames.cap) {
+        st.d_wtiles.reset(); st.d_frames.reset(); st.eval_pending = false;
+        if (st.d_wtiles.grow(pl.wtile_bytes) != hipSuccess || st.d_frames.grow(pl.frame_bytes) != hipSuccess) {
+            (void)hipGetLastError();
+            batch_err(b, "shared-rig evaluation: scratch allocation (%zu bytes) failed", pl.wtile_bytes + pl.frame_bytes);
+            return FD_E_NOMEM;
+        }
+    }
+    const int rc = wait_last_eval(b, "shared-rig evaluation", stream, &st.eval_pending, st.eval_done);
+    if (rc) return rc;
+    t.wtiles = st.d_wtiles; t.frames = st.d_frames;
+    t.nF = b->n; t.nslot = pl.nslot; t.ntiles = pl.ntiles; t.nkb = pl.nkb;
+    t.poly_at = pl.poly_at; t.copy_at = pl.copy_at; t.norm_at = pl.norm_at;
+    for (int i = 0; i < b->n; ++i) { t.P_out[i] = b->fold_P_out[i]; t.falloff_out[i] = b->fold_fall ? b->fold_fall[i] : nullptr; }
+    *set_out = si;
+    return 1;
+}
+
 int fd_batch_prepare_shared(fd_batch *b, void *hip_stream, float *const *d_P_out, float *const *d_falloff_out)
 {
     if (!b || !d_P_out) return FD_E_INVALID;
@@ -3102,11 +3160,14 @@
     b->lean = lean;
     FD_COOK_TICK();
     if (events) mark(events->before_build, bs);
-    if ((rc = fd_batch_build_async(b, build_stream))) return rc;
+    if (lean) { b->fold_P_out = d_P_out; b->fold_fall = d_falloff_out; }
+    rc = fd_batch_build_async(b, build_stream);
+    b->fold_P_out = nullptr; b->fold_fall = nullptr;
+    if (rc) return rc;
     scope.built = true;
     if (events) mark(events->after_build, bs);
     FD_COOK_TICK();
-    if ((rc = fd_batch_prepare_shared(b, build_stream, d_P_out, d_falloff_out))) return rc;
+    if (!(lean && b->prepared) && (rc = fd_batch_prepare_shared(b, build_stream, d_P_out, d_falloff_out))) return rc;
     FD_COOK_TICK();
     if (es != bs) {
         if (!b->group_ev.make() || hipEventRecord(b->group_ev, bs) != hipSuccess || hipStreamWaitEvent(es, b->group_ev, 0) != hipSuccess) {
diff --git a/facedeform_amd/csrc/fd_eval_shared.hip b/facedeform_amd/csrc/fd_eval_shared.hip
--- a/facedeform_amd/csrc/fd_eval_shared.hip
+++ b/facedeform_amd/csrc/fd_eval_shared.hip
@@ -5,6 +5,7 @@
 
 #include "fd_eval_common.h"
 #include "fd_shared_common.h"
+#include "fd_shared_pack.h"
 #include "fd_shared_plan.h"
 
 namespace fd {
@@ -548,30 +549,14 @@
     const int kb = blockIdx.x, T = blockIdx.y, NT = gridDim.y;
     const int w16 = wide_w16(NT);
     if (T == 0) {
-        uint2 *dst = reinterpret_cast<uint2 *>(wtiles + copy_at) + (size_t)kb * 128;
         if (gauss) {
             if (threadIdx.x < 32) {
                 const int centre = 32 * kb + (int)threadIdx.x;
                 wtiles[copy_at + (size_t)kb * 64 + threadIdx.x] =
                     centre < Mpad ? *reinterpret_cast<const uint4 *>(&slots.rec32[0][centre]) : make_uint4(0u, 0u, 0u, 0u);
             }
-        } else if (layout == 1) {
-            if (threadIdx.x < 64) {
-                const int lane = threadIdx.x, h = lane >> 5, r = lane & 31;
-                const int tile = 2 * kb + (r >> 4);
-                uint4 v = make_uint4(0u, 0u, 0u, 0u);
-                if (tile < Mpad / 16) {
-                    const unsigned *a0 = ctiles[tile].a[16 * (2 * h) + (r & 15)], *a1 = ctiles[tile].a[16 * (2 * h + 1) + (r & 15)];
-                    v = make_uint4(a0[0], a0[1], a1[0], a1[1]);
-                }
-                wtiles[copy_at + (size_t)kb * 64 + lane] = v;
-            }
-        } else if (threadIdx.x < 128) {
-            const int i = threadIdx.x >> 6, lane = threadIdx.x & 63, h = lane >> 5, r = lane & 31;
-            const int tile = 2 * kb + (r >> 4);
-            uint2 v = make_uint2(0u, 0u);
-            if (tile < Mpad / 16) { const unsigned *a = ctiles[tile].a[16 * (2 * i + h) + (r & 15)]; v = make_uint2(a[0], a[1]); }
-            dst[threadIdx.x] = v;
+        } else {
+            wide_pack_centres(wtiles, copy_at, kb, (int)threadIdx.x, ctiles, Mpad, layout);
         }
         if (kb == 0 && threadIdx.x == 255) {
             const float *nn = slots.model[0]->norm32;
@@ -588,9 +573,7 @@
         for (int off = 4; off >= 1; off >>= 1) m = fmaxf(m, __shfl_xor(m, off));
         const bool same_rig = (kb == 0 && T == 0) ? rig_matches(slots, f, nslot, l, 8) : true;
         if (l == 0) {
-            int k = 0;
-            if (m > 0.f && m < INFINITY) k = 13 - (__builtin_amdgcn_frexp_expf(m) - 1);
-            k = k < -100 ? -100 : (k > 100 ? 100 : k);
+            const int k = wide_scale_exp(m);
             s_scale[f] = ldexpf(1.f, k);
             if (kb == 0 && T == 0) {
                 SharedFrame fr;
@@ -605,46 +588,13 @@
     }
     __syncthreads();
     if (threadIdx.x >= 128) return;
-    const int s = threadIdx.x >> 6, lane = threadIdx.x & 63, h = lane >> 5;
+    const int s = threadIdx.x >> 6, lane = threadIdx.x & 63;
     int f, c;
-    if (layout == 1) {
-        const int rho = lane & 31, k = 16 * T + 4 * (rho >> 3) + (rho & 3);
-        f = 2 * (k / 3) + ((rho >> 2) & 1); c = k % 3;
-    } else {
-        const int row = 32 * T + (lane & 31);
-        f = row / 3; c = row % 3;
-    }
+    wide_row(layout, T, lane & 31, f, c);
     const bool live = f < nslot;
     const float sc = live ? s_scale[f] : 0.f;
-    f16x8 hi, lo;
-#pragma unroll
-    for (int m = 0; m < 8; ++m) {
-        const int centre = 32 * kb + 8 * (2 * s + (m >> 2)) + 4 * h + (m & 3);
-        float w = 0.f;
-        if (live && centre < Mpad) {
-            const Rec32 r = slots.rec32[f][centre];
-            w = (c == 0 ? r.wx : (c == 1 ? r.wy : r.wz)) * sc;
-        }
-        const _Float16 hh = (_Float16)w;
-        hi[m] = hh;
-        lo[m] = (_Float16)(w - (float)hh);
-    }
-    uint4 *dst = wtiles + (size_t)kb * w16 + (size_t)((T * 2 + s) * 2) * 64;
-    dst[lane] = __builtin_bit_cast(uint4, hi);
-    dst[64 + lane] = __builtin_bit_cast(uint4, lo);
-    if (kb == 0 && s == 0) {
-        f16x8 pt;
-#pragma unroll
-        for (int m = 0; m < 8; ++m) {
-            const int coef = h == 0 ? (m < 5 ? m : m - 4) : (m == 0 ? 4 : (m < 6 ? m - 1 : -1));
-            const bool want_lo = h == 1 && m >= 1;
-            float w = 0.f;
-            if (live && coef >= 0) w = slots.model[f]->poly32[5 * c + coef] * sc;
-            const _Float16 hh = (_Float16)w;
-            pt[m] = want_lo ? (_Float16)(w - (float)hh) : hh;
-        }
-        wtiles[poly_at + (size_t)T * 64 + lane] = __builtin_bit_cast(uint4, pt);
-    }
+    wide_pack_weights(wtiles, w16, kb, T, s, lane, live ? slots.rec32[f] : nullptr, c, live, sc, Mpad);
+    if (kb == 0 && s == 0) wide_pack_poly(wtiles, poly_at, T, lane, live ? slots.model[f]->poly32 : nullptr, c, live, sc);
 }
 
 constexpr int kWideVpm = 3;
diff --git a/facedeform_amd/csrc/fd_internal.h b/facedeform_amd/csrc/fd_internal.h
--- a/facedeform_amd/csrc/fd_internal.h
+++ b/facedeform_amd/csrc/fd_internal.h
@@ -149,7 +149,14 @@
 hipError_t launch_build_spd(const BuildBuffers &b, hipStream_t stream, hipEvent_t ev_mid);
 hipError_t launch_resolve_spd(const BuildBuffers &b, hipStream_t stream, const PointSrc *src);
 bool reg_applicable(int kind, int term, double lambda, int M);
-hipError_t launch_build_reg(const BuildBuffers &b, hipStream_t stream, const PointSrc *src, hipEvent_t ev_mid);
+struct TailShared {
+    void *wtiles, *frames;
+    int nF, nslot, ntiles, nkb;
+    size_t poly_at, copy_at, norm_at;
+    float *P_out[kMaxBatch], *falloff_out[kMaxBatch];
+};
+hipError_t launch_build_reg(const BuildBuffers &b, hipStream_t stream, const PointSrc *src, hipEvent_t ev_mid,
+                            const TailShared *fold = nullptr, bool *folded = nullptr);
 hipError_t launch_build_reg_shared(const BuildBuffers &b, hipStream_t stream, const PointSrc *src, hipEvent_t ev_mid, double *fac);
 size_t reg_factor_doubles();
 hipError_t reg_build_init();
diff --git a/facedeform_amd/csrc/fd_pack.h b/facedeform_amd/csrc/fd_pack.h
--- a/facedeform_amd/csrc/fd_pack.h
+++ b/facedeform_amd/csrc/fd_pack.h
@@ -117,21 +117,18 @@
     return kind == FD_KERNEL_THIN_PLATE ? 0.5 : (kind == FD_KERNEL_BIHARMONIC ? -1.0 : 1.0);
 }
 
+struct PackNorm {
+    double x0[3], sc, inv_s, w32, w64, kappa, rad_o, dmax, dmin;
+};
+constexpr int kPackNormDoubles = 11;
+static_assert(sizeof(PackNorm) == kPackNormDoubles * sizeof(double), "stored as doubles (fd_build_reg.hip: the front buffer)");
+constexpr int kPackRedDoubles = 4 * 18;
+
 template <class Src>
-__device__ __forceinline__ void pack_body_from(const Src &in, const BatchSlot &slot, int , int M, int Mpad, int T, int kind, int from_w, int layers)
-{
-    double *W = slot.W;
-    Rec32 *rec32 = slot.rec32;
-    Rec64 *rec64 = slot.rec64;
-    DevModel *model = slot.model;
-    __shared__ int s_bad;
-    __shared__ double s_red[4 * 18];
+__device__ __forceinline__ PackNorm pack_normalise(const Src &in, int M, int kind, double *s_red)
+{
     const int tid = threadIdx.x;
-    if (tid == 0) s_bad = 0;
-    __syncthreads();
     const double kLn2 = 0.6931471805599453;
-    const double kLog2e = 1.4426950408889634;
-    const bool gauss = kind == FD_KERNEL_GAUSSIAN || kind == FD_KERNEL_GAUSSIAN_QNN;
 
     double sx = 0.0, sy = 0.0, sz = 0.0;
     for (int j = tid; j < M; j += 256) { sx += in.centre(j, 0); sy += in.centre(j, 1); sz += in.centre(j, 2); }
@@ -184,6 +181,27 @@
     if (kind == FD_KERNEL_THIN_PLATE) { w32 = 0.5 * kLn2 * sc * sc; w64 = 0.5; kappa = sc * sc * log(sc); }
     if (kind == FD_KERNEL_BIHARMONIC) { w32 = -sc; w64 = -1.0; }
     if (kind == FD_KERNEL_CUBIC) { w32 = sc * sc * sc; }
+    PackNorm nm;
+    nm.x0[0] = x0[0]; nm.x0[1] = x0[1]; nm.x0[2] = x0[2];
+    nm.sc = sc; nm.inv_s = inv_s; nm.w32 = w32; nm.w64 = w64; nm.kappa = kappa; nm.rad_o = rad_o;
+    nm.dmax = sqrt(ext[2]); nm.dmin = dl ? sqrt(-ext[3]) : 0.0;
+    return nm;
+}
+
+template <class Src>
+__device__ __forceinline__ void pack_records(const Src &in, const PackNorm &nm, const BatchSlot &slot, int M, int Mpad, int T, int kind,
+                                             int from_w, int layers, int *s_bad_p, double *s_red)
+{
+    double *W = slot.W;
+    Rec32 *rec32 = slot.rec32;
+    Rec64 *rec64 = slot.rec64;
+    DevModel *model = slot.model;
+    int &s_bad = *s_bad_p;
+    const int tid = threadIdx.x;
+    const double kLog2e = 1.4426950408889634;
+    const bool gauss = kind == FD_KERNEL_GAUSSIAN || kind == FD_KERNEL_GAUSSIAN_QNN;
+    const double x0[3] = {nm.x0[0], nm.x0[1], nm.x0[2]};
+    const double sc = nm.sc, inv_s = nm.inv_s, w32 = nm.w32, w64 = nm.w64, kappa = nm.kappa, rad_o = nm.rad_o;
 
     bool bad = false;
     float wmax = 0.f;
@@ -260,7 +278,7 @@
             const double v = m[15 + c] * phimax + poly;
             S = v > S ? v : S;
         }
-        const double dmax = sqrt(ext[2]), dmin = dl ? sqrt(-ext[3]) : 0.0;
+        const double dmax = nm.dmax, dmin = nm.dmin;
         model->fp32_error = S * 2.98023223876953125e-08;
         model->cancellation = dmax > 0.0 ? S / dmax : 0.0;
         model->delta_min = dmin;
@@ -277,6 +295,17 @@
         model->terminationtype = tt;
         if (slot.host_status) *slot.host_status = tt;
     }
+}
+
+template <class Src>
+__device__ __forceinline__ void pack_body_from(const Src &in, const BatchSlot &slot, int , int M, int Mpad, int T, int kind, int from_w, int layers)
+{
+    __shared__ int s_bad;
+    __shared__ double s_red[kPackRedDoubles];
+    if (threadIdx.x == 0) s_bad = 0;
+    __syncthreads();
+    const PackNorm nm = pack_normalise(in, M, kind, s_red);
+    pack_records(in, nm, slot, M, Mpad, T, kind, from_w, layers, &s_bad, s_red);
 }
 
 __device__ __forceinline__ void pack_body(const BatchSlot &slot, int npad, int M, int Mpad, int T, int kind, int from_w, int layers)
diff --git a/facedeform_amd/csrc/fd_shared_pack.h b/facedeform_amd/csrc/fd_shared_pack.h
--- /dev/null
+++ b/facedeform_amd/csrc/fd_shared_pack.h
@@ -0,0 +1,87 @@
+#pragma once
+#include "fd_shared_common.h"
+
+namespace fd {
+namespace {
+
+__device__ __forceinline__ void wide_row(int layout, int T, int rho, int &f, int &c)
+{
+    if (layout == 1) {
+        const int k = 16 * T + 4 * (rho >> 3) + (rho & 3);
+        f = 2 * (k / 3) + ((rho >> 2) & 1); c = k % 3;
+    } else {
+        const int row = 32 * T + rho;
+        f = row / 3; c = row % 3;
+    }
+}
+
+__device__ __forceinline__ int wide_scale_exp(float m)
+{
+    int k = 0;
+    if (m > 0.f && m < INFINITY) k = 13 - (__builtin_amdgcn_frexp_expf(m) - 1);
+    return k < -100 ? -100 : (k > 100 ? 100 : k);
+}
+
+__device__ __forceinline__ void wide_pack_weights(uint4 *wtiles, int w16, int kb, int T, int s, int lane, const Rec32 *rec, int c, bool live,
+                                                  float sc, int Mpad)
+{
+    const int h = lane >> 5;
+    f16x8 hi, lo;
+#pragma unroll
+    for (int m = 0; m < 8; ++m) {
+        const int centre = 32 * kb + 8 * (2 * s + (m >> 2)) + 4 * h + (m & 3);
+        float w = 0.f;
+        if (live && centre < Mpad) {
+            const Rec32 r = rec[centre];
+            w = (c == 0 ? r.wx : (c == 1 ? r.wy : r.wz)) * sc;
+        }
+        const _Float16 hh = (_Float16)w;
+        hi[m] = hh;
+        lo[m] = (_Float16)(w - (float)hh);
+    }
+    uint4 *dst = wtiles + (size_t)kb * w16 + (size_t)((T * 2 + s) * 2) * 64;
+    dst[lane] = __builtin_bit_cast(uint4, hi);
+    dst[64 + lane] = __builtin_bit_cast(uint4, lo);
+}
+
+__device__ __forceinline__ void wide_pack_poly(uint4 *wtiles, size_t poly_at, int T, int lane, const float *poly32, int c, bool live, float sc)
+{
+    const int h = lane >> 5;
+    f16x8 pt;
+#pragma unroll
+    for (int m = 0; m < 8; ++m) {
+        const int coef = h == 0 ? (m < 5 ? m : m - 4) : (m == 0 ? 4 : (m < 6 ? m - 1 : -1));
+        const bool want_lo = h == 1 && m >= 1;
+        float w = 0.f;
+        if (live && coef >= 0) w = poly32[5 * c + coef] * sc;
+        const _Float16 hh = (_Float16)w;
+        pt[m] = want_lo ? (_Float16)(w - (float)hh) : hh;
+    }
+    wtiles[poly_at + (size_t)T * 64 + lane] = __builtin_bit_cast(uint4, pt);
+}
+
+__device__ __forceinline__ void wide_pack_centres(uint4 *wtiles, size_t copy_at, int kb, int t, const MfmaTileH *ctiles, int Mpad, int layout)
+{
+    if (layout == 1) {
+        if (t < 64) {
+            const int lane = t, h = lane >> 5, r = lane & 31;
+            const int tile = 2 * kb + (r >> 4);
+            uint4 v = make_uint4(0u, 0u, 0u, 0u);
+            if (tile < Mpad / 16) {
+                const unsigned *a0 = ctiles[tile].a[16 * (2 * h) + (r & 15)], *a1 = ctiles[tile].a[16 * (2 * h + 1) + (r & 15)];
+                v = make_uint4(a0[0], a0[1], a1[0], a1[1]);
+            }
+            wtiles[copy_at + (size_t)kb * 64 + lane] = v;
+        }
+    } else if (t < 128) {
+        uint2 *dst = reinterpret_cast<uint2 *>(wtiles + copy_at) + (size_t)kb * 128;
+        const int i = t >> 6, lane = t & 63, h = lane >> 5, r = lane & 31;
+        const int tile = 2 * kb + (r >> 4);
+        uint2 v = make_uint2(0u, 0u);
+        if (tile < Mpad / 16) { const unsigned *a = ctiles[tile].a[16 * (2 * i + h) + (r & 15)]; v = make_uint2(a[0], a[1]); }
+        dst[t] = v;
+    }
+}
+
+}
+}
```

New measurement: 51200. 0.902x the previous value.
